# esw0116/DynaVSR

Hardware: AMD Instinct MI355X
Metric: inner-loop frames/sec/GPU (EDVR-M x4, 5x3x180x320): forward leg = BASELINE.json configs[1]; the inner MAML step and the per-frame pipeline are `inner_step` / `per_frame_pipeline` (higher is better)
Workload: dtype f32; 1 GPU; EDVR-M x4 forward (PCD deformable alignment + TSA fusion + reconstruction), clips of 1x5x3x180x320 -> 3x720x1280 (BASELINE.json configs[1]); one step = 2 clip(s) per GPU, one per HIP stream (adapt.super_resolve_video); clips_in_flight_per_gpu=2

## Files before the change

### dynavsr_amd/_lib.py

```python
import ctypes
import os
from ctypes import POINTER, Structure, c_char_p, c_float, c_int, c_longlong, c_size_t, c_void_p

import torch

_runtime = {"configured": False, "hw_queues": None, "effective": None}


def configure_runtime(hw_queues=6):
    if not _runtime["configured"]:
        user = os.environ.get("GPU_MAX_HW_QUEUES")
        late = torch.cuda.is_initialized()
        if user is None and not late:
            os.environ["GPU_MAX_HW_QUEUES"] = str(int(hw_queues))
        _runtime.update(configured=True, hw_queues=os.environ.get("GPU_MAX_HW_QUEUES"),
                        effective=(user is not None) or not late)
    return {"hw_queues": _runtime["hw_queues"], "effective": _runtime["effective"]}


def runtime_report(device=None):
    r = configure_runtime()
    overlaps = None
    if torch.cuda.is_available():
        with torch.cuda.device(device if device is not None else torch.cuda.current_device()):
            overlaps = int(lib().dvsr_side_stream_overlaps(stream()))
    return {"hw_queues": r["hw_queues"], "effective": r["effective"], "side_stream_overlaps": overlaps}


_HERE = os.path.dirname(os.path.abspath(__file__))
SO_PATH = os.path.join(_HERE, "libdynavsr_hip.so")
_lib = None

ACT_NONE, ACT_LRELU, ACT_RELU = 0, 1, 2


class Conv2dDesc(Structure):
    _fields_ = [("x0", c_void_p), ("x1", c_void_p), ("w", c_void_p), ("bias", c_void_p),
                ("res", c_void_p), ("y", c_void_p),
                ("N", c_int), ("c0", c_int), ("c1", c_int), ("H", c_int), ("W", c_int),
                ("Cout", c_int), ("ks", c_int), ("stride", c_int), ("pad", c_int), ("act", c_int),
                ("pixel_shuffle", c_int), ("x1_bdiv", c_int),
                ("x0_bstride", c_longlong), ("x1_bstride", c_longlong),
                ("pre", c_void_p), ("pre_bdiv", c_int)]


class EdvrConfig(Structure):
    _fields_ = [(k, c_int) for k in ("nf", "nframes", "groups", "front_RBs", "back_RBs", "scale",
                                     "center", "bf16_mfma")]


class FrameDesc(Structure):
    _fields_ = [("format", c_int), ("h", c_int), ("w", c_int), ("row_stride", c_longlong), ("plane_stride", c_longlong),
                ("pixel_stride", c_int)]


FRAME_F32_CHW, FRAME_U8_HWC_RGB, FRAME_U8_HWC_BGR, FRAME_U8_Y = 0, 1, 2, 3
FRAME_U16_Y_MSB, FRAME_U16_Y_10, FRAME_U16_Y_12 = 4, 5, 6
FRAME_PAD_REFLECT, FRAME_PAD_REPLICATE = 0, 1


class YuvDesc(Structure):
    _fields_ = [("format", c_int), ("h", c_int), ("w", c_int), ("matrix", c_int), ("range", c_int),
                ("plane", c_void_p * 3), ("row_stride", c_longlong * 3)]


YUV_NV12, YUV_I420 = 0, 1
YUV_BT601, YUV_BT709 = 0, 1
YUV_LIMITED, YUV_FULL = 0, 1


class Yuv16Desc(Structure):
    _fields_ = [("format", c_int), ("depth", c_int), ("h", c_int), ("w", c_int), ("matrix", c_int), ("range", c_int),
                ("plane", c_void_p * 3), ("row_stride", c_longlong * 3)]


YUV16_SEMI_MSB, YUV16_PLANAR_LSB = 0, 1


class ResizeAxis(Structure):
    _fields_ = [("first", c_void_p), ("weights", c_void_p), ("taps", c_int)]


FLIP_W, FLIP_H = 1, 2


class EstimatorConfig(Structure):
    _fields_ = [(k, c_int) for k in ("kind", "nf", "in_nc", "scale", "nframes")]


def _declare(lib):
    P, I, F, LL = c_void_p, c_int, c_float, c_longlong
    sig = {
        "dvsr_last_error": (c_char_p, []),
        "dvsr_version": (I, []),
        "dvsr_mdcn_forward": (I, [P] * 6 + [I] * 13 + [P]),
        "dvsr_mdcn_forward_fast_workspace_bytes": (c_size_t, [I, I, I]),
        "dvsr_mdcn_forward_fast": (I, [P] * 6 + [I] * 7 + [P, c_size_t, P]),
        "dvsr_mdcn_pack_forward": (I, [P] * 5 + [I] * 13 + [P]),
        "dvsr_conv2d_forward": (I, [POINTER(Conv2dDesc), P]),
        "dvsr_upsample_bilinear_forward": (I, [P, P, LL, I, I, I, F, P]),
        "dvsr_upsample_bilinear_backward": (I, [P, P, LL, I, I, I, F, I, P]),
        "dvsr_pool3s2_forward": (I, [P, P, P, LL, I, I, P]),
        "dvsr_pool3s2_backward": (I, [P, P, P, P, LL, I, I, P]),
        "dvsr_tsa_gate_forward": (I, [P] * 5 + [I, I, I, LL, P]),
        "dvsr_tsa_gate_backward": (I, [P] * 8 + [I, I, I, LL, P]),
        "dvsr_tsa_blend_forward": (I, [P] * 4 + [LL, P]),
        "dvsr_tsa_blend_backward": (I, [P] * 5 + [LL, P]),
        "dvsr_edvr_plan_create": (I, [POINTER(EdvrConfig), I, I, I, POINTER(c_void_p)]),
        "dvsr_edvr_plan_create_grouped": (I, [POINTER(EdvrConfig), I, I, I, I, POINTER(c_void_p)]),
        "dvsr_edvr_plan_create_ex": (I, [POINTER(EdvrConfig), I, I, I, I, I, POINTER(c_void_p)]),
        "dvsr_edvr_plan_destroy": (None, [P]),
        "dvsr_edvr_num_params": (I, [P]),
        "dvsr_edvr_num_launches": (I, [P]),
        "dvsr_edvr_workspace_bytes": (c_size_t, [P, I]),
        "dvsr_edvr_forward": (I, [P, POINTER(c_void_p), P, P, P, c_size_t, P]),
        "dvsr_edvr_forward_packed": (I, [P, POINTER(c_void_p), P, P, P, c_size_t, P]),
        "dvsr_edvr_backward": (I, [P, POINTER(c_void_p), P, P, POINTER(c_void_p), P, P, c_size_t, P]),
        "dvsr_edvr_num_backward_launches": (I, [P]),
        "dvsr_estimator_plan_create": (I, [POINTER(EstimatorConfig), I, I, I, POINTER(c_void_p)]),
        "dvsr_estimator_plan_create_grouped": (I, [POINTER(EstimatorConfig), I, I, I, I, POINTER(c_void_p)]),
        "dvsr_estimator_plan_create_ex": (I, [POINTER(EstimatorConfig), I, I, I, I, I, POINTER(c_void_p)]),
        "dvsr_estimator_plan_destroy": (None, [P]),
        "dvsr_estimator_num_params": (I, [P]),
        "dvsr_estimator_num_launches": (I, [P, I]),
        "dvsr_estimator_workspace_bytes": (c_size_t, [P, I]),
        "dvsr_estimator_forward": (I, [P, POINTER(c_void_p), P, P, P, c_size_t, P]),
        "dvsr_estimator_backward": (I, [P, POINTER(c_void_p), P, P, POINTER(c_void_p), P, c_size_t, P]),
        "dvsr_conv2d_backward_workspace_bytes": (c_size_t, [POINTER(Conv2dDesc)]),
        "dvsr_conv2d_backward": (I, [POINTER(Conv2dDesc), P, P, P, P, P, P, c_size_t, P]),
        "dvsr_mdcn_backward_workspace_bytes": (c_size_t, [I] * 10),
        "dvsr_mdcn_backward": (I, [P] * 10 + [I] * 12 + [P, c_size_t, P]),
        "dvsr_adam_step": (I, [POINTER(c_void_p)] * 4 + [POINTER(LL), I, F, F, F, F, F, I, P]),
        "dvsr_sgd_step": (I, [POINTER(c_void_p)] * 2 + [POINTER(LL), I, F, F, P]),
        "dvsr_replicate_tensors": (I, [POINTER(c_void_p)] * 2 + [POINTER(LL), I, I, P]),
        "dvsr_degrade_apply": (I, [P, P, P, I, I, I, I, I, I, I, I, I, P]),
        "dvsr_frame_metrics_workspace_bytes": (c_size_t, [I, I, I]),
        "dvsr_frame_metrics": (I, [P, P, I, I, I, F, F, P, P, P, c_size_t, P]),
        "dvsr_charbonnier_workspace_bytes": (c_size_t, []),
        "dvsr_charbonnier_forward": (I, [P, P, P, LL, F, P, c_size_t, P]),
        "dvsr_conv2d_packed_workspace_bytes": (c_size_t, [POINTER(Conv2dDesc)]),
        "dvsr_conv2d_forward_packed": (I, [POINTER(Conv2dDesc), P, c_size_t, P]),
        "dvsr_conv2d_dgrad_packed": (I, [POINTER(Conv2dDesc), P, P, P, c_size_t, P]),
        "dvsr_conv2d_packed_geometry": (I, [POINTER(Conv2dDesc), POINTER(ctypes.c_int * 4)]),
        "dvsr_conv2d_wgrad_geometry": (I, [POINTER(Conv2dDesc), I, I, POINTER(ctypes.c_int * 8)]),
        "dvsr_conv2d_wgrad_workspace_bytes": (c_size_t, [POINTER(Conv2dDesc), I]),
        "dvsr_conv2d_wgrad_bf16": (I, [POINTER(Conv2dDesc), P, P, P, P, c_size_t, P]),
        "dvsr_conv2d_wgrad_split3": (I, [POINTER(Conv2dDesc), P, P, P, P, c_size_t, P]),
        "dvsr_flow_warp_forward": (I, [P, P, P, I, I, I, I, LL, P]),
        "dvsr_flow_warp_backward": (I, [P, P, P, P, P, I, I, I, I, LL, P]),
        "dvsr_avgpool2_forward": (I, [P, P, LL, I, I, P]),
        "dvsr_avgpool2_backward": (I, [P, P, LL, I, I, I, P]),
        "dvsr_resize_bilinear_ac_forward": (I, [P, P, LL, I, I, I, I, F, LL, P]),
        "dvsr_resize_bilinear_ac_backward": (I, [P, P, LL, I, I, I, I, F, LL, P]),
        "dvsr_upsample_bicubic_ac_forward": (I, [P, P, LL, I, I, I, P]),
        "dvsr_upsample_bicubic_ac_backward": (I, [P, P, LL, I, I, I, P]),
        "dvsr_channel_affine": (I, [P, P, P, P, I, I, LL, LL, LL, I, P]),
        "dvsr_batchnorm_workspace_bytes": (c_size_t, [I]),
        "dvsr_batchnorm_forward": (I, [P] * 8 + [I, I, LL, I, F, F, I, P, c_size_t, P]),
        "dvsr_batchnorm_backward": (I, [P] * 9 + [I, I, LL, I, I, P, c_size_t, P]),
        "dvsr_temporal_gather3_forward": (I, [P, P, I, I, I, LL, I, P]),
        "dvsr_temporal_gather3_backward": (I, [P, P, I, I, I, LL, I, P]),
        "dvsr_dynamic_filter_forward": (I, [P, P, P, P, I, I, I, I, I, P]),
        "dvsr_dynamic_filter_backward": (I, [P, P, P, P, P, P, I, I, I, I, I, P]),
        "dvsr_conv3x3_small_cout": (I, [P, P, P, P, P, I, I, I, I, I, I, P]),
        "dvsr_conv1x1_dual": (I, [P, P, P, P, P, P, P, I, I, I, I, I, P]),
        "dvsr_patch_gather_forward": (I, [P, P, POINTER(c_int), POINTER(c_int), I, I, I, I, I, I, P]),
        "dvsr_patch_gather_backward": (I, [P, P, POINTER(c_int), POINTER(c_int), I, I, I, I, I, I, P]),
        "dvsr_l1_tail_forward": (I, [P, P, P, F, P, LL, P, c_size_t, P]),
        "dvsr_l1_tail_backward": (I, [P, P, P, F, P, LL, P]),
        "dvsr_charbonnier_backward": (I, [P, P, P, P, LL, F, P]),
        "dvsr_charbonnier_forward_grouped": (I, [P, P, P, LL, I, F, P, c_size_t, P]),
        "dvsr_charbonnier_backward_grouped": (I, [P, P, P, P, LL, I, F, P]),
        "dvsr_l1_tail_forward_grouped": (I, [P, P, P, F, P, LL, I, P, c_size_t, P]),
        "dvsr_l1_tail_backward_grouped": (I, [P, P, P, F, P, LL, I, P]),
        "dvsr_edvr_op_info": (I, [P, I, c_char_p, I, c_char_p, I, POINTER(ctypes.c_double),
                                  POINTER(ctypes.c_double)]),
        "dvsr_edvr_forward_timed": (I, [P, POINTER(c_void_p), P, P, P, c_size_t, P, POINTER(c_float)]),
        "dvsr_debug_mfma_peak": (LL, [P, I, I, I, I, P]),
        "dvsr_debug_mfma_shadow": (I, [P, P, I, I, I, I, I, P]),
        "dvsr_edvr_tensor_info": (I, [P, c_char_p, POINTER(LL), POINTER(LL)]),
        "dvsr_edvr_plan_work": (I, [P, POINTER(ctypes.c_double * 9)]),
        "dvsr_edvr_plan_work_nograd": (I, [P, POINTER(ctypes.c_double * 9)]),
        "dvsr_edvr_op_launch_count": (I, [P, I, I]),
        "dvsr_side_stream_overlaps": (I, [P]),
        "dvsr_edvr_op_output": (I, [P, I, I, POINTER(c_int), POINTER(LL), POINTER(LL)]),
        "dvsr_estimator_plan_work": (I, [P, POINTER(ctypes.c_double * 9)]),
        "dvsr_edvr_stream_create": (I, [POINTER(EdvrConfig), I, I, I, POINTER(c_void_p)]),
        "dvsr_edvr_stream_destroy": (None, [P]),
        "dvsr_edvr_stream_num_params": (I, [P]),
        "dvsr_edvr_stream_num_launches": (I, [P, I]),
        "dvsr_edvr_stream_cache_bytes": (c_size_t, [P]),
        "dvsr_edvr_stream_workspace_bytes": (c_size_t, [P]),
        "dvsr_edvr_stream_extract": (I, [P, POINTER(c_void_p), P, I, P, c_size_t, P, c_size_t, I, P]),
        "dvsr_edvr_stream_fuse": (I, [P, POINTER(c_void_p), POINTER(c_int), P, c_size_t, P, P, c_size_t, I, P]),
        "dvsr_frame_ingest": (I, [P, POINTER(FrameDesc), P, I, I, I, P]),
        "dvsr_frame_emit": (I, [P, I, I, P, POINTER(FrameDesc), F, F, P]),
        "dvsr_edvr_stream_extract_frame": (I, [P, POINTER(c_void_p), P, POINTER(FrameDesc), I, I, P, c_size_t, P, c_size_t, I,
                                               P]),
        "dvsr_frame_ingest_yuv": (I, [POINTER(YuvDesc), P, I, I, I, P]),
        "dvsr_frame_emit_yuv": (I, [P, I, I, POINTER(YuvDesc), F, F, P]),
        "dvsr_edvr_stream_extract_frame_yuv": (I, [P, POINTER(c_void_p), POINTER(YuvDesc), I, I, P, c_size_t, P, c_size_t, I, P]),
        "dvsr_frame_luma_sad": (I, [P, P, POINTER(FrameDesc), LL, I, P, P]),
        "dvsr_frame_ingest_yuv16": (I, [POINTER(Yuv16Desc), P, I, I, I, P]),
        "dvsr_frame_emit_yuv16": (I, [P, I, I, POINTER(Yuv16Desc), F, F, P]),
        "dvsr_edvr_stream_extract_frame_yuv16": (I, [P, POINTER(c_void_p), POINTER(Yuv16Desc), I, I, P, c_size_t, P, c_size_t, I,
                                                     P]),
        "dvsr_frame_resize_taps": (I, [I, I]),
        "dvsr_frame_resize_table": (I, [I, I, I, P, P]),
        "dvsr_frame_resize": (I, [P, I, I, I, I, P, I, I, I, I, POINTER(ResizeAxis), POINTER(ResizeAxis), P]),
        "dvsr_frame_flip": (I, [P, P, LL, I, I, I, P]),
        "dvsr_frame_flip_mean": (I, [P, P, P, P, P, LL, I, I, P]),
    }
    for name, (res, args) in sig.items():
        fn = getattr(lib, name)
        fn.restype = res
        fn.argtypes = args
    return sig


def lib():
    global _lib
    if _lib is None:
        if not os.path.exists(SO_PATH):
            raise RuntimeError(
                "libdynavsr_hip.so is missing (%s). Build it with `python -m dynavsr_amd.build` "
                "(hipcc --offload-arch=gfx950); there is no fallback path." % SO_PATH)
        _lib = ctypes.CDLL(os.environ.get("DVSR_HIP_LIB", SO_PATH))
        _lib._signatures = _declare(_lib)
    return _lib


def check(rc, what=""):
    if rc != 0:
        msg = lib().dvsr_last_error().decode("utf-8", "replace")
        raise RuntimeError("libdynavsr_hip %s failed (rc=%d): %s" % (what, rc, msg))


def ptr(t):
    if t is None:
        return None
    if not t.is_cuda:
        raise RuntimeError("libdynavsr_hip needs a tensor on the GPU, got device %s" % t.device)
    if t.dtype != torch.float32:
        raise RuntimeError("libdynavsr_hip computes in fp32, got %s" % t.dtype)
    if not t.is_contiguous():
        raise RuntimeError("libdynavsr_hip needs contiguous tensors")
    return t.data_ptr()


def stream():
    return torch.cuda.current_stream().cuda_stream
```

### dynavsr_amd/csrc/conv_small.hip

```cpp
#include "common.h"
#include "kernels.h"

namespace dvsr {

struct SmallK {
  const float* x; const float* w; const float* bias; const float* res; float* y;
  int N, C, H, W, Cout, act, tiles_x, tiles_y, ntiles;
  int wdiv; long long w_gs; int b_gs;
};

typedef float f32x2 __attribute__((ext_vector_type(2)));

template <int COUT>
__global__ __launch_bounds__(256) void conv3x3_small_cout_kernel(SmallK a) {
  constexpr int CC = 8, TH = 8, TW = 64, IH = TH + 2, IW = TW + 2, PLANE = IH * IW, E = (PLANE + 255) / 256;
  constexpr int WPC = ((9 * COUT + 3) / 4) * 4;
  __shared__ __attribute__((aligned(16))) float s_in[2][CC * PLANE];
  extern __shared__ __attribute__((aligned(16))) float s_w[];
  const int tpx = (a.ntiles + 7) >> 3;
  const int tile = (blockIdx.x & 7) * tpx + (blockIdx.x >> 3);
  if ((int)(blockIdx.x >> 3) >= tpx || tile >= a.ntiles) return;
  const int tx_ = tile % a.tiles_x;
  const int t2 = tile / a.tiles_x;
  const int ty_ = t2 % a.tiles_y;
  const int n = t2 / a.tiles_y;
  const int oy0 = ty_ * TH, ox0 = tx_ * TW;
  const int tid = threadIdx.x;
  const int py = tid >> 5, px2 = (tid & 31) * 2;
  const size_t HW = (size_t)a.H * a.W;
  const float* xn = a.x + (size_t)n * a.C * HW;
  const float* wn = wset_ptr(a.w, a.w_gs, n, a.wdiv);
  const float* bn = wset_ptr(a.bias, a.b_gs, n, a.wdiv);

  unsigned eoff[E];
  bool evalid[E];
#pragma unroll
  for (int e = 0; e < E; ++e) {
    const int idx = tid + 256 * e;
    const int iy = idx / IW, ix = idx - iy * IW;
    const int gy = oy0 - 1 + iy, gx = ox0 - 1 + ix;
    evalid[e] = idx < PLANE && (unsigned)gy < (unsigned)a.H && (unsigned)gx < (unsigned)a.W;
    eoff[e] = evalid[e] ? (unsigned)(gy * a.W + gx) * 4u : 0u;
  }
  f32x2 acc[COUT];
#pragma unroll
  for (int o = 0; o < COUT; ++o) acc[o] = f32x2{0.f, 0.f};
  float rin[CC][E];
  const int nch = ceil_div(a.C, CC);
  for (int i = tid; i < nch * CC * WPC; i += 256) {
    const int ci = i / WPC, r = i - ci * WPC;
    const int tap = r / COUT, o = r - tap * COUT;
    s_w[i] = (ci < a.C && tap < 9) ? wn[((size_t)o * a.C + ci) * 9 + tap] : 0.f;
  }
  auto prefetch = [&](int k) {
#pragma unroll
    for (int c = 0; c < CC; ++c) {
      const int ci = k * CC + c;
      const char* src = reinterpret_cast<const char*>(xn + (size_t)(ci < a.C ? ci : 0) * HW);
#pragma unroll
      for (int e = 0; e < E; ++e) rin[c][e] = *reinterpret_cast<const float*>(src + eoff[e]);
    }
  };
  prefetch(0);
  for (int k = 0; k < nch; ++k) {
    float* s = s_in[k & 1];
#pragma unroll
    for (int c = 0; c < CC; ++c)
#pragma unroll
      for (int e = 0; e < E; ++e) {
        const int idx = tid + 256 * e;
        if (e + 1 < E || idx < PLANE) s[c * PLANE + idx] = (evalid[e] && k * CC + c < a.C) ? rin[c][e] : 0.f;
      }
    __syncthreads();
    if (k + 1 < nch) prefetch(k + 1);
    const float* p0 = s + py * IW + px2;
#pragma unroll
    for (int c = 0; c < CC; ++c) {
      f32x4 wq[WPC / 4];
#pragma unroll
      for (int q = 0; q < WPC / 4; ++q)
        wq[q] = *reinterpret_cast<const f32x4*>(s_w + (size_t)(k * CC + c) * WPC + 4 * q);
#pragma unroll
      for (int ty = 0; ty < 3; ++ty) {
        const f32x2 lo = *reinterpret_cast<const f32x2*>(p0 + c * PLANE + ty * IW);
        const f32x2 hi = *reinterpret_cast<const f32x2*>(p0 + c * PLANE + ty * IW + 2);
        const float v[4] = {lo[0], lo[1], hi[0], hi[1]};
#pragma unroll
        for (int tx = 0; tx < 3; ++tx)
#pragma unroll
          for (int o = 0; o < COUT; ++o) {
            const int wi = (ty * 3 + tx) * COUT + o;
            const float wv = wq[wi >> 2][wi & 3];
            acc[o] = __builtin_elementwise_fma(f32x2{wv, wv}, f32x2{v[tx], v[tx + 1]}, acc[o]);
          }
      }
    }
  }
  const int oy = oy0 + py, ox = ox0 + px2;
  if (oy >= a.H || ox >= a.W) return;
  const bool two = ox + 1 < a.W;
  float bvs[COUT];
  f32x2 rvs[COUT];
#pragma unroll
  for (int o = 0; o < COUT; ++o) {
    bvs[o] = bn ? bn[o] : 0.f;
    const size_t idx = ((size_t)n * a.Cout + o) * HW + (size_t)oy * a.W + ox;
    rvs[o] = (a.res && two && (idx & 1) == 0) ? *reinterpret_cast<const f32x2*>(a.res + idx) : f32x2{0.f, 0.f};
  }
#pragma unroll
  for (int o = 0; o < COUT; ++o) {
    const float bv = bvs[o];
    f32x2 v = {apply_act(acc[o][0] + bv, a.act), apply_act(acc[o][1] + bv, a.act)};
    const size_t idx = ((size_t)n * a.Cout + o) * HW + (size_t)oy * a.W + ox;
    if (two && (idx & 1) == 0) {
      v += rvs[o];
      *reinterpret_cast<f32x2*>(a.y + idx) = v;
    } else {
      a.y[idx] = v[0] + (a.res ? a.res[idx] : 0.f);
      if (two) a.y[idx + 1] = v[1] + (a.res ? a.res[idx + 1] : 0.f);
    }
  }
}

struct SmallMfmaShape {
  static constexpr int TH = 6, TW = 56, RH = 8, RW = 64, X0 = 4, NPOS = RH * RW, APITCH = 68;
  static constexpr size_t LDS_BYTES = (size_t)(32 * APITCH + 27 * NPOS) * sizeof(float);
};

__device__ __forceinline__ __amdgpu_buffer_rsrc_t sm_rsrc(const float* base) {
  return __builtin_amdgcn_make_buffer_rsrc(const_cast<float*>(base), 0, 0x7fffffff, 0x00020000);
}
__device__ __forceinline__ f32x4 sm_load16(__amdgpu_buffer_rsrc_t rs, unsigned voff, unsigned soff) {
  return __builtin_bit_cast(f32x4, __builtin_amdgcn_raw_buffer_load_b128(rs, (int)voff, (int)soff, 0));
}

template <int COUT>
__global__ __launch_bounds__(256, 2) void conv3x3_small_cout_mfma_kernel(SmallK a) {
  using Sh = SmallMfmaShape;
  constexpr int TH = Sh::TH, TW = Sh::TW, RW = Sh::RW, NPOS = Sh::NPOS, AP = Sh::APITCH, NM = 9 * COUT;
  extern __shared__ __attribute__((aligned(16))) float s_mf[];
  float* const s_a = s_mf;
  float* const s_p = s_mf + 32 * AP;
  const int tpx = (a.ntiles + 7) >> 3;
  const int tile = (blockIdx.x & 7) * tpx + (blockIdx.x >> 3);
  if ((int)(blockIdx.x >> 3) >= tpx || tile >= a.ntiles) return;
  const int tx_ = tile % a.tiles_x;
  const int t2 = tile / a.tiles_x;
  const int ty_ = t2 % a.tiles_y;
  const int n = t2 / a.tiles_y;
  const int oy0 = ty_ * TH, ox0 = tx_ * TW;
  const int tid = threadIdx.x, lane = tid & 63;
  const int wave = __builtin_amdgcn_readfirstlane(tid >> 6);
  const int nn = lane & 31, kk = lane >> 5;
  const unsigned HW4 = (unsigned)a.H * a.W * 4u;
  const float* wn = wset_ptr(a.w, a.w_gs, n, a.wdiv);
  const float* bn = wset_ptr(a.bias, a.b_gs, n, a.wdiv);

  const int gy = oy0 - 1 + 2 * wave + (nn >> 4), gx = ox0 - Sh::X0 + 4 * (nn & 15);
  const bool inimg = (unsigned)gy < (unsigned)a.H && (unsigned)gx < (unsigned)a.W;
  const unsigned voff = inimg ? (unsigned)(8 * kk) * HW4 + (unsigned)(gy * a.W + gx) * 4u : 0x80000000u;
  const __amdgpu_buffer_rsrc_t xrs = sm_rsrc(a.x + (size_t)n * 64 * a.H * a.W);
  f32x4 B[2][16];
  auto issue = [&](int half) __attribute__((always_inline)) {
#pragma unroll
    for (int s = 0; s < 16; ++s) {
      const int c = 16 * (2 * half + (s >> 3)) + (s & 7);
      B[half][s] = sm_load16(xrs, voff, (unsigned)c * HW4);
    }
  };
  issue(0);
  for (int i = tid; i < 32 * 64; i += 256) {
    const int m = i >> 6, c = i & 63;
    const int tap = m / COUT, o = m - tap * COUT;
    s_a[m * AP + c] = m < NM ? wn[((size_t)o * 64 + c) * 9 + tap] : 0.f;
  }
  issue(1);
  __syncthreads();
  f32x4 A[8];
#pragma unroll
  for (int q = 0; q < 8; ++q) A[q] = *reinterpret_cast<const f32x4*>(s_a + nn * AP + 16 * (q >> 1) + 8 * kk + 4 * (q & 1));

  f32x16 acc[4];
#pragma unroll
  for (int j = 0; j < 4; ++j)
#pragma unroll
    for (int r = 0; r < 16; ++r) acc[j][r] = 0.f;
#pragma unroll
  for (int half = 0; half < 2; ++half)
#pragma unroll
    for (int s = 0; s < 16; ++s) {
      const int ch = 2 * half + (s >> 3), i = s & 7;
      const float av = A[2 * ch + (i >> 2)][i & 3];
#pragma unroll
      for (int j = 0; j < 4; ++j) acc[j] = __builtin_amdgcn_mfma_f32_32x32x2f32(av, B[half][s][j], acc[j], 0, 0, 0);
    }

#pragma unroll
  for (int r = 0; r < 16; ++r) {
    const int m = (r & 3) + 8 * (r >> 2) + 4 * kk;
    if (m < NM)
      *reinterpret_cast<f32x4*>(s_p + m * NPOS + 128 * wave + 4 * nn) = f32x4{acc[0][r], acc[1][r], acc[2][r], acc[3][r]};
  }
  __syncthreads();

  if (tid >= TH * (TW / 2)) return;
  const int y = tid / (TW / 2), xp = (tid - y * (TW / 2)) * 2;
  const int oy = oy0 + y, ox = ox0 + xp;
  if (oy >= a.H || ox >= a.W) return;
  float s0[COUT], s1[COUT];
#pragma unroll
  for (int o = 0; o < COUT; ++o) { s0[o] = 0.f; s1[o] = 0.f; }
#pragma unroll
  for (int dy = 0; dy < 3; ++dy) {
    const float* row = s_p + (y + dy) * RW + xp + Sh::X0 - 1;
#pragma unroll
    for (int dx = 0; dx < 3; ++dx)
#pragma unroll
      for (int o = 0; o < COUT; ++o) {
        const float* pm = row + ((dy * 3 + dx) * COUT + o) * NPOS + dx;
        s0[o] += pm[0];
        s1[o] += pm[1];
      }
  }
  const size_t HW = (size_t)a.H * a.W;
#pragma unroll
  for (int o = 0; o < COUT; ++o) {
    const float bv = bn ? bn[o] : 0.f;
    f32x2 v = {apply_act(s0[o] + bv, a.act), apply_act(s1[o] + bv, a.act)};
    const size_t idx = ((size_t)n * a.Cout + o) * HW + (size_t)oy * a.W + ox;
    if (a.res) v += *reinterpret_cast<const f32x2*>(a.res + idx);
    *reinterpret_cast<f32x2*>(a.y + idx) = v;
  }
}

template <int COUT>
static int launch_small_mfma(SmallK k, hipStream_t st) {
  using Sh = SmallMfmaShape;
  k.tiles_x = ceil_div(k.W, Sh::TW); k.tiles_y = ceil_div(k.H, Sh::TH); k.ntiles = k.tiles_x * k.tiles_y * k.N;
  auto kern = conv3x3_small_cout_mfma_kernel<COUT>;
  static PerDeviceOnce once;
  set_dyn_lds_once(once, (const void*)kern, Sh::LDS_BYTES);
  hipLaunchKernelGGL(kern, dim3(8 * ceil_div(k.ntiles, 8)), dim3(256), Sh::LDS_BYTES, st, k);
  return check_launch("conv3x3_small_cout_mfma_kernel");
}

int conv3x3_small_cout_run(const float* x, const float* w, const float* bias, const float* res, float* y, int N,
                           int C, int H, int W, int Cout, int act, hipStream_t st, int wdiv, long long w_gs, int b_gs) {
  DVSR_REQUIRE(x && w && y && Cout >= 1 && Cout <= 4, DVSR_ERR_INVALID, "conv3x3_small_cout: bad argument");
  SmallK k;
  k.x = x; k.w = w; k.bias = bias; k.res = res; k.y = y; k.N = N; k.C = C; k.H = H; k.W = W; k.Cout = Cout; k.act = act;
  k.wdiv = wdiv > 0 ? wdiv : 1; k.w_gs = w_gs; k.b_gs = b_gs;
  static const bool mfma_on = [] { const char* v = getenv("DVSR_CONV_LAST_MFMA"); return v && v[0] == '1'; }();
  if (mfma_on && C == 64 && Cout <= 3 && W % 4 == 0 && (unsigned long long)C * H * W * 4 < 0x7fffffffull &&
      ((((uintptr_t)x | (uintptr_t)y | (uintptr_t)res) & 15) == 0) && w_gs % 4 == 0) {
    if (Cout == 1) return launch_small_mfma<1>(k, st);
    if (Cout == 2) return launch_small_mfma<2>(k, st);
    return launch_small_mfma<3>(k, st);
  }
  k.tiles_x = ceil_div(W, 64); k.tiles_y = ceil_div(H, 8); k.ntiles = k.tiles_x * k.tiles_y * N;
  auto wbytes = [&](int cout) { return (size_t)ceil_div(C, 8) * 8 * (((9 * cout + 3) / 4) * 4) * sizeof(float); };
  switch (Cout) {
    case 1: hipLaunchKernelGGL(conv3x3_small_cout_kernel<1>, dim3(8 * ceil_div(k.ntiles, 8)), dim3(256), wbytes(1), st, k); break;
    case 2: hipLaunchKernelGGL(conv3x3_small_cout_kernel<2>, dim3(8 * ceil_div(k.ntiles, 8)), dim3(256), wbytes(2), st, k); break;
    case 3: hipLaunchKernelGGL(conv3x3_small_cout_kernel<3>, dim3(8 * ceil_div(k.ntiles, 8)), dim3(256), wbytes(3), st, k); break;
    default: hipLaunchKernelGGL(conv3x3_small_cout_kernel<4>, dim3(8 * ceil_div(k.ntiles, 8)), dim3(256), wbytes(4), st, k); break;
  }
  return check_launch("conv3x3_small_cout_kernel");
}

}

extern "C" int dvsr_conv3x3_small_cout(const float* x, const float* w, const float* bias, const float* res, float* y, int N,
                                       int C, int H, int W, int Cout, int act, dvsr_stream_t stream) {
  DVSR_REQUIRE(N > 0 && C > 0 && H > 0 && W > 0, DVSR_ERR_INVALID, "conv3x3_small_cout: empty tensor");
  return dvsr::conv3x3_small_cout_run(x, w, bias, res, y, N, C, H, W, Cout, act, (hipStream_t)stream, 1, 0, 0);
}
```

### dynavsr_amd/csrc/engine.hip

```cpp
#include <algorithm>
#include <cstdlib>
#include <string>
#include <vector>

#include "common.h"
#include "kernels.h"
#include "small_grid.h"

namespace dvsr {

enum { SP_ARENA = 0, SP_INPUT = 1, SP_OUTPUT = 2, SP_NONE = 3 };
struct T {
  int space = SP_NONE;
  size_t off = 0, numel = 0;
  bool valid() const { return space != SP_NONE; }
};

enum OpType { OP_CONV, OP_DCN, OP_UP, OP_POOL, OP_GATE, OP_BLEND, OP_ADD, OP_PAD, OP_MEANSUB, OP_ADDMEAN };

struct Op {
  OpType type;
  const char* name = "";
  T x0, x1, res, y, y2;
  int pw = -1, pb = -1;
  int N = 0, c0 = 0, c1 = 0, H = 0, W = 0, Cout = 0, ks = 3, stride = 1, act = 0, ps = 0;
  int x1_bdiv = 1, dg = 8;
  int pad = -1;
  int pmode = 0, T = 1;
  int wmap = 0;
  size_t w2_off = 0;
  int no_dgrad = 0;
  int pad_out = 0;
  struct T ypad;
  int fused_into = -1;
  int dual = -1;
  long long x0_bs = 0, x1_bs = 0;
  int S = 1;
  float mul = 1.f;
  size_t planes = 0;
  int gB = 0, gN = 0, gC = 0;
  size_t gHW = 0;
  struct PackSlot { ConvGeo geo = {8, 8, 2}; size_t off = 0, floats = 0; };
  PackSlot dgrad[2], dcn_pack;
  enum LaunchRole { WHOLE, MAIN_PART, REF_PART };
  struct Launch { PackSlot pack; int c_off = 0, c = 0; LaunchRole role = WHOLE; };
  struct LaunchList {
    int n = 0; Launch l[2];
    const Launch* begin() const { return l; }
    const Launch* end() const { return l + n; }
    const Launch& primary() const { return l[n - 1]; }
  } launches[2];
  struct T pre;
};
enum FwdMode { FWD_GRAD = 0, FWD_NOGRAD = 1 };

enum { R_ACT = 0, R_GRAD = 1, R_X = 2, R_GX = 3, R_GOUT = 4, R_TMP = 5, R_NONE = 6 };
struct Ref {
  int space = R_NONE;
  size_t off = 0;
};
enum BType { B_MEMSET, B_COPYADD, B_ACT, B_WGRAD, B_DGRAD, B_REDUCE, B_DCN, B_UP, B_POOL, B_GATE, B_BLEND,
             B_PADFOLD, B_ADDMEAN, B_WUNMAP };
struct BOp {
  BType type;
  int fwd = -1;
  Ref a, b, c, d, e, f;
  size_t n = 0;
  int accum = 0, which = 0, cnt = 1, B = 0;
  int mask_op = -1;
  size_t ws_off = 0, ws_bytes = 0;
  long long bs = 0;
  size_t per = 0;
};

static inline int conv_pad(const Op& o) { return o.pad < 0 ? o.ks / 2 : o.pad; }
static inline int conv_out(const Op& o, int in) { return (in + 2 * conv_pad(o) - o.ks) / o.stride + 1; }

}

struct dvsr_edvr_plan {
  dvsr_edvr_config cfg;
  int B, H, W;
  int n_params = 0;
  size_t arena_floats = 0;
  std::vector<dvsr::Op> ops;
  std::vector<std::pair<std::string, dvsr::T>> named;
  std::vector<std::pair<size_t, size_t>> allocs;
  std::vector<dvsr::BOp> bops;
  size_t dpack_floats = 0;
  bool use_v1 = false;
  size_t tmp_floats = 0;
  size_t scratch_bytes = 0;
  size_t wscratch_bytes = 0;
  mutable hipStream_t side = nullptr;
  mutable hipEvent_t ev_fork = nullptr, ev_join = nullptr;
  int side_streams = 1;
  int fork_every = 3;
  const char* bwd_unsupported = nullptr;
  int wgroups = 1;
  int wsets = 1;
  bool split_any_pad = false;
};

namespace dvsr {

static T arena_alloc(dvsr_edvr_plan& p, const char* name, size_t numel) {
  T t;
  t.space = SP_ARENA;
  t.off = p.arena_floats;
  t.numel = numel;
  p.allocs.emplace_back(t.off, numel);
  p.arena_floats += (numel + 63) & ~(size_t)63;
  if (name && *name) p.named.emplace_back(name, t);
  return t;
}

static WgradDesc wgrad_shape(const dvsr_edvr_plan& p, const Op& o, int which) {
  WgradDesc d;
  d.x_bs = which ? o.x1_bs : o.x0_bs; d.x_bdiv = which ? o.x1_bdiv : 1; d.gy_ps = o.ps;
  d.N = o.N; d.Cin = which ? o.c1 : o.c0; d.H = o.H; d.W = o.W; d.Cout = o.Cout;
  d.Ctot = o.c0 + o.c1; d.c_off = which ? o.c0 : 0;
  d.ks = o.ks; d.stride = o.stride; d.pad = conv_pad(o);
  d.groups = p.wgroups; d.dW_gs = (long long)o.Cout * (o.c0 + o.c1) * o.ks * o.ks; d.db_gs = o.Cout;
  d.mode = (p.cfg.bf16_mfma == 1 && !o.wmap) ? 1 : (wgrad_split3_default() ? 2 : 0);
  return d;
}

static Op::LaunchList plan_hoist(const Op& o, const dvsr_edvr_plan& p, ConvAllow fwd_ok, const Op::Launch& whole) {
  Op::LaunchList pair;
  const char* hv = getenv("DVSR_PCD_HOIST");
  if ((hv && hv[0] == '0') || p.use_v1 || p.wsets != 1 || whole.pack.geo.kernel != ConvKernel::WINO_F4 || o.x1_bdiv <= 1 || o.c1 <= 0 ||
      o.N % o.x1_bdiv != 0 || o.res.valid() || o.ps)
    return pair;
  const int Ho = conv_out(o, o.H), Wo = conv_out(o, o.W), bd = o.x1_bdiv;
  const ConvAllow shared = fwd_ok | ALLOW_WINO_F4 | ALLOW_SHARED_DEVICE;
  const ConvAllow only_f4 = without(fwd_ok, ALLOW_KSPLIT) | ALLOW_WINO_F4 | ALLOW_ONLY_F4;
  auto choose = [&](int n, int c, ConvAllow allow) { return conv2_choose(o.ks, o.stride, n, Ho, Wo, o.Cout, c, allow); };
  auto f4 = [](const ConvGeo& g) { return g.kernel == ConvKernel::WINO_F4; };
  const ConvGeo gm = choose(o.N, o.c0, shared), gr = choose(o.N / bd, o.c1, only_f4);
  const ConvGeo u1 = choose(bd, o.c0 + o.c1, shared), m1 = choose(bd, o.c0, shared), r1 = choose(1, o.c1, only_f4);
  if (f4(gm) && f4(gr) && f4(u1) && f4(m1) && f4(r1) &&
      conv2_f4_occupied_cycles(bd, Ho, Wo, o.Cout, o.c0, m1.th) + conv2_f4_occupied_cycles(1, Ho, Wo, o.Cout, o.c1, r1.th) <
          conv2_f4_occupied_cycles(bd, Ho, Wo, o.Cout, o.c0 + o.c1, u1.th)) {
    const size_t mf = conv2_pack_floats(o.ks, o.Cout, o.c0, gm), rf = conv2_pack_floats(o.ks, o.Cout, o.c1, gr);
    if (mf + rf <= whole.pack.floats)
      pair = {2, {{{gr, whole.pack.off + mf, rf}, o.c0, o.c1, Op::REF_PART}, {{gm, whole.pack.off, mf}, 0, o.c0, Op::MAIN_PART}}};
  }
  return pair;
}

static void plan_conv_launches(Op& o, dvsr_edvr_plan& p) {
  const int ks = o.ks, N = o.N, c0 = o.c0, c1 = o.c1, Cout = o.Cout, Ho = conv_out(o, o.H), Wo = conv_out(o, o.W);
  const char* s2 = getenv("DVSR_EST_SPLIT2");
  const int split2 = s2 ? atoi(s2) : 1;
  const bool bf = p.cfg.bf16_mfma && (ks == 3 || (ks == 2 && p.split_any_pad && p.cfg.bf16_mfma == 2 && split2 && c0 % 16 == 0)) &&
                  o.stride == 1 && (o.pad < 0 || p.split_any_pad) && (c1 == 0 || c0 % 16 == 0);
  static const int split_th8_from = getenv("DVSR_SPLIT_TH8_FROM") ? atoi(getenv("DVSR_SPLIT_TH8_FROM")) : 200;
  auto as_bf = [&](ConvGeo g, int ho, int wo, int cout, bool dgrad = false) {
    if (!bf || (ks == 2 && split2 == 2 && dgrad)) return g;
    if (ks == 2 && (long long)ceil_div(wo, 32) * ceil_div(ho, 4) * N * ceil_div(cout, 64) < 256) return g;
    g.cc = 16; g.th = 4; g.bf = p.cfg.bf16_mfma == 2 ? 2 : 1;
    if (g.bf == 2 && (long long)ceil_div(wo, 32) * ceil_div(ho, 8) * N * ceil_div(cout, 32 * g.mt) >= split_th8_from)
      g.th = 8;
    return g;
  };
  const bool plain = o.pad < 0 && !o.wmap && !p.cfg.bf16_mfma;
  const ConvAllow ks_ok = (plain && (c1 == 0 || c0 % 32 == 0) ? ALLOW_KSPLIT : ALLOW_NONE) |
                          (plain && c0 % 8 == 0 && c1 % 8 == 0 ? ALLOW_DMA_HALO | ALLOW_WINO : ALLOW_NONE);
  const ConvAllow fwd_ok = (o.ps == 0 || (o.ps == 2 && !o.res.valid())) ? ks_ok : without(ks_ok, ALLOW_WINO);
  auto whole = [&](const ConvGeo& g) {
    const size_t floats = conv2_pack_floats(ks, Cout, c0 + c1, g);
    return Op::Launch{{g, arena_alloc(p, "", floats * p.wsets).off, floats}, 0, c0 + c1, Op::WHOLE};
  };
  o.launches[FWD_GRAD] = {1, {whole(as_bf(conv2_choose(ks, o.stride, N, Ho, Wo, Cout, c0 + c1, fwd_ok), Ho, Wo, Cout))}};
  Op::LaunchList& nograd = o.launches[FWD_NOGRAD] = o.launches[FWD_GRAD];
  if ((fwd_ok & ALLOW_WINO) && !nograd.l[0].pack.geo.bf) {
    const ConvGeo g5 = conv2_choose(ks, o.stride, N, Ho, Wo, Cout, c0 + c1, fwd_ok | ALLOW_WINO_F4 | ALLOW_SHARED_DEVICE);
    if (g5.kernel == ConvKernel::WINO_F4) nograd.l[0] = whole(g5);
  }
  const Op::LaunchList pair = plan_hoist(o, p, fwd_ok, nograd.l[0]);
  if (pair.n) {
    o.pre = arena_alloc(p, "", (size_t)(N / o.x1_bdiv) * Cout * Ho * Wo);
    nograd = pair;
  }
  for (int which = 0; which < 2; ++which) {
    const int ci = which ? c1 : c0;
    if (!ci) continue;
    Op::PackSlot& dg = o.dgrad[which];
// ... 71 lines not shown

enum PlanPart { PART_WHOLE = 0, PART_EXTRACT = 1, PART_FUSE = 2 };

struct SlotLayout { size_t off[3], numel[3], raw, floats; };
static SlotLayout slot_layout(int C, int H, int W) {
  auto up = [](size_t n) { return (n + 63) & ~(size_t)63; };
  SlotLayout s;
  s.numel[0] = (size_t)C * H * W; s.numel[1] = (size_t)C * (H / 2) * (W / 2); s.numel[2] = (size_t)C * (H / 4) * (W / 4);
  s.off[0] = 0; s.off[1] = up(s.numel[0]); s.off[2] = s.off[1] + up(s.numel[1]);
  s.raw = s.off[2] + up(s.numel[2]);
  s.floats = s.raw + up((size_t)3 * H * W);
  return s;
}

static int build_plan(dvsr_edvr_plan& p, PlanPart part = PART_WHOLE) {
  const dvsr_edvr_config& c = p.cfg;
  const int B = p.B, Nf = c.nframes, C = c.nf, H = p.H, W = p.W, BN = B * Nf, dg = c.groups;
  const int H2 = H / 2, W2 = W / 2, H4 = H / 4, W4 = W / 4;
  const size_t HW = (size_t)H * W, HW2 = (size_t)H2 * W2, HW4 = (size_t)H4 * W4;
  Builder b(p);
  const int L = ACT_LRELU, R = ACT_RELU, NO = ACT_NONE;
  T none;
  const int EN = part == PART_EXTRACT ? 1 : BN;
  T xin; xin.space = SP_INPUT; xin.off = 0; xin.numel = (size_t)EN * 3 * HW;

  T f1, f2, f3;
  if (part == PART_FUSE) {
    f1 = b.alloc("L1_fea", (size_t)BN * C * HW);
    f2 = b.alloc("L2_fea", (size_t)BN * C * HW2);
    f3 = b.alloc("L3_fea", (size_t)BN * C * HW4);
    b.pcur += 2 * (1 + 2 * c.front_RBs + 4);
  } else {
    const SlotLayout sl = slot_layout(C, H, W);
    auto dst = [&](int l, bool final_of_level) {
      T t;
      if (part == PART_EXTRACT && final_of_level) { t.space = SP_OUTPUT; t.off = sl.off[l]; t.numel = sl.numel[l]; }
      return t;
    };
    f1 = b.conv("conv_first", b.take(), xin, 3, none, 0, EN, H, W, C, 3, 1, L, none, 0, 1, 0, 0, dst(0, c.front_RBs == 0));
    for (int i = 0; i < c.front_RBs; ++i) {
      auto p1 = b.take(); auto p2 = b.take();
      T t = b.conv("fe_rb_a", p1, f1, C, none, 0, EN, H, W, C, 3, 1, R);
      f1 = b.conv("fe_rb_b", p2, t, C, none, 0, EN, H, W, C, 3, 1, NO, f1, 0, 1, 0, 0, dst(0, i == c.front_RBs - 1));
    }
    p.named.emplace_back("L1_fea", f1);
    f2 = b.conv("fea_L2_conv1", b.take(), f1, C, none, 0, EN, H, W, C, 3, 2, L);
    f2 = b.conv("L2_fea", b.take(), f2, C, none, 0, EN, H2, W2, C, 3, 1, L, none, 0, 1, 0, 0, dst(1, true));
    f3 = b.conv("fea_L3_conv1", b.take(), f2, C, none, 0, EN, H2, W2, C, 3, 2, L);
    f3 = b.conv("L3_fea", b.take(), f3, C, none, 0, EN, H4, W4, C, 3, 1, L, none, 0, 1, 0, 0, dst(2, true));
  }
  if (part == PART_EXTRACT) {
    p.n_params = b.pcur;
    return DVSR_OK;
  }

  struct DP { int w, b; Builder::CP com; };
  auto take_dcn = [&]() { DP d; d.w = b.pcur; d.b = b.pcur + 1; b.pcur += 2; d.com = b.take(); return d; };
  auto L3o1 = b.take(); auto L3o2 = b.take(); DP L3d = take_dcn();
  auto L2o1 = b.take(); auto L2o2 = b.take(); auto L2o3 = b.take(); DP L2d = take_dcn(); auto L2f = b.take();
  auto L1o1 = b.take(); auto L1o2 = b.take(); auto L1o3 = b.take(); DP L1d = take_dcn(); auto L1f = b.take();
  auto cso1 = b.take(); auto cso2 = b.take(); DP csd = take_dcn();
  const int ctr = c.center;
  T ref1 = Builder::view(f1, (size_t)ctr * C * HW, 0), ref2 = Builder::view(f2, (size_t)ctr * C * HW2, 0),
    ref3 = Builder::view(f3, (size_t)ctr * C * HW4, 0);
  const long long rs1 = (long long)Nf * C * HW, rs2 = (long long)Nf * C * HW2, rs3 = (long long)Nf * C * HW4;
  T o3 = b.conv("L3_offset_conv1", L3o1, f3, C, ref3, C, BN, H4, W4, C, 3, 1, L, none, 0, Nf, 0, rs3);
  o3 = b.conv("L3_offset", L3o2, o3, C, none, 0, BN, H4, W4, C, 3, 1, L);
  T om3 = b.conv("L3_om", L3d.com, o3, C, none, 0, BN, H4, W4, dg * 27, 3, 1, NO);
  T fe3 = b.dcn("L3_aligned", L3d.w, L3d.b, f3, om3, BN, C, H4, W4, dg, L);
  T o2 = b.conv("L2_offset_conv1", L2o1, f2, C, ref2, C, BN, H2, W2, C, 3, 1, L, none, 0, Nf, 0, rs2);
  T u3 = b.up("L3_offset_up", o3, (size_t)BN * C, H4, W4, 2, 2.f);
  o2 = b.conv("L2_offset_conv2", L2o2, o2, C, u3, C, BN, H2, W2, C, 3, 1, L);
  o2 = b.conv("L2_offset", L2o3, o2, C, none, 0, BN, H2, W2, C, 3, 1, L);
  T om2 = b.conv("L2_om", L2d.com, o2, C, none, 0, BN, H2, W2, dg * 27, 3, 1, NO);
  T d2 = b.dcn("L2_dcn", L2d.w, L2d.b, f2, om2, BN, C, H2, W2, dg, NO);
  T uf3 = b.up("L3_aligned_up", fe3, (size_t)BN * C, H4, W4, 2, 1.f);
  T fe2 = b.conv("L2_aligned", L2f, d2, C, uf3, C, BN, H2, W2, C, 3, 1, L);
  T o1 = b.conv("L1_offset_conv1", L1o1, f1, C, ref1, C, BN, H, W, C, 3, 1, L, none, 0, Nf, 0, rs1);
  T u2 = b.up("L2_offset_up", o2, (size_t)BN * C, H2, W2, 2, 2.f);
  o1 = b.conv("L1_offset_conv2", L1o2, o1, C, u2, C, BN, H, W, C, 3, 1, L);
  o1 = b.conv("L1_offset", L1o3, o1, C, none, 0, BN, H, W, C, 3, 1, L);
  T om1 = b.conv("L1_om", L1d.com, o1, C, none, 0, BN, H, W, dg * 27, 3, 1, NO);
  T d1 = b.dcn("L1_dcn", L1d.w, L1d.b, f1, om1, BN, C, H, W, dg, NO);
  T uf2 = b.up("L2_aligned_up", fe2, (size_t)BN * C, H2, W2, 2, 1.f);
  T fe1 = b.conv("L1_aligned", L1f, d1, C, uf2, C, BN, H, W, C, 3, 1, NO);
  T oc = b.conv("cas_offset_conv1", cso1, fe1, C, ref1, C, BN, H, W, C, 3, 1, L, none, 0, Nf, 0, rs1);
  oc = b.conv("cas_offset", cso2, oc, C, none, 0, BN, H, W, C, 3, 1, L);
  T omc = b.conv("cas_om", csd.com, oc, C, none, 0, BN, H, W, dg * 27, 3, 1, NO);
  T aligned = b.dcn("aligned", csd.w, csd.b, fe1, omc, BN, C, H, W, dg, L);

  auto tA1 = b.take(); auto tA2 = b.take(); auto ffu = b.take(); auto s1 = b.take(); auto s2 = b.take();
  auto s3 = b.take(); auto s4 = b.take(); auto s5 = b.take(); auto sL1 = b.take(); auto sL2 = b.take();
  auto sL3 = b.take(); auto sa1 = b.take(); auto sa2 = b.take();
  T emb_ref = b.conv("tsa_emb_ref", tA2, Builder::view(aligned, (size_t)ctr * C * HW, 0), C, none, 0, B, H,
                     W, C, 3, 1, NO, none, 0, 1, (long long)Nf * C * HW);
  T emb = b.conv("tsa_emb", tA1, aligned, C, none, 0, BN, H, W, C, 3, 1, NO);
  T cor = b.alloc("tsa_cor", (size_t)BN * HW);
  T gated = b.alloc("tsa_gated", (size_t)BN * C * HW);
  {
    Op o; o.type = OP_GATE; o.name = "tsa_gate"; o.x0 = emb; o.x1 = emb_ref; o.res = aligned;
    o.y = cor; o.y2 = gated; o.gB = B; o.gN = Nf; o.gC = C; o.gHW = HW;
    p.ops.push_back(o);
  }
  T fea = b.conv("tsa_fea", ffu, gated, Nf * C, none, 0, B, H, W, C, 1, 1, L);
  T att = b.conv("tsa_att1", s1, gated, Nf * C, none, 0, B, H, W, C, 1, 1, L);
  {
    static const bool dual_on = [] { const char* v = getenv("DVSR_TSA_DUAL"); return !(v && v[0] == '0'); }();
    const int ia = (int)p.ops.size() - 2, ib = ia + 1;
    if (dual_on && C == 64 && !p.cfg.bf16_mfma) { p.ops[ia].dual = ib; p.ops[ib].fused_into = ia; }
  }
  T pmx, pav;
  b.pool("tsa_pool1", att, (size_t)B * C, H, W, pmx, pav);
  att = b.conv("tsa_att2", s2, pmx, C, pav, C, B, H2, W2, C, 1, 1, L);
  T attL = b.conv("tsa_attL1", sL1, att, C, none, 0, B, H2, W2, C, 1, 1, L);
  T qmx, qav;
  b.pool("tsa_pool2", attL, (size_t)B * C, H2, W2, qmx, qav);
  attL = b.conv("tsa_attL2", sL2, qmx, C, qav, C, B, H4, W4, C, 3, 1, L);
  attL = b.conv("tsa_attL3", sL3, attL, C, none, 0, B, H4, W4, C, 3, 1, L);
  T attLu = b.up("tsa_attL_up", attL, (size_t)B * C, H4, W4, 2, 1.f);
  T a3 = b.conv("tsa_att3", s3, att, C, none, 0, B, H2, W2, C, 3, 1, L);
  T att3 = b.alloc("tsa_att3_sum", (size_t)B * C * HW2);
  {
    Op o; o.type = OP_ADD; o.name = "tsa_att3_add"; o.x0 = a3; o.x1 = attLu; o.y = att3;
    p.ops.push_back(o);
  }
  T a4 = b.conv("tsa_att4", s4, att3, C, none, 0, B, H2, W2, C, 1, 1, L);
  T a4u = b.up("tsa_att4_up", a4, (size_t)B * C, H2, W2, 2, 1.f);
  T a5 = b.conv("tsa_att", s5, a4u, C, none, 0, B, H, W, C, 3, 1, NO);
  T ad = b.conv("tsa_add1", sa1, a5, C, none, 0, B, H, W, C, 1, 1, L);
  ad = b.conv("tsa_add2", sa2, ad, C, none, 0, B, H, W, C, 1, 1, NO);
  T out = b.alloc("tsa_out", (size_t)B * C * HW);
  {
    Op o; o.type = OP_BLEND; o.name = "tsa_blend"; o.x0 = fea; o.x1 = a5; o.res = ad; o.y = out;
    p.ops.push_back(o);
  }

  for (int i = 0; i < c.back_RBs; ++i) {
    auto p1 = b.take(); auto p2 = b.take();
    T t = b.conv("rc_rb_a", p1, out, C, none, 0, B, H, W, C, 3, 1, R);
    out = b.conv("rc_rb_b", p2, t, C, none, 0, B, H, W, C, 3, 1, NO, out);
  }
  p.named.emplace_back("recon", out);
  int h = H, w = W;
  if (c.scale == 4) {
    out = b.conv("upconv1", b.take(), out, C, none, 0, B, h, w, C * 4, 3, 1, L, none, 2);
    h *= 2; w *= 2;
    out = b.conv("upconv2", b.take(), out, C, none, 0, B, h, w, 256, 3, 1, L, none, 2);
  } else {
    out = b.conv("upconv2", b.take(), out, C, none, 0, B, h, w, 256, 3, 1, L, none, 2);
  }
  h *= 2; w *= 2;
  out = b.conv("HRconv", b.take(), out, 64, none, 0, B, h, w, 64, 3, 1, L);
  T base = b.alloc("base", (size_t)B * 3 * h * w);
  for (int bi = 0; bi < B; ++bi) {
    Op o; o.type = OP_UP; o.name = "base_up";
    o.x0 = Builder::view(xin, part == PART_FUSE ? 0 : ((size_t)bi * Nf + ctr) * 3 * HW, 3 * HW);
    o.planes = 3; o.H = H; o.W = W; o.S = c.scale; o.mul = 1.f;
    o.y = Builder::view(base, (size_t)bi * 3 * h * w, (size_t)3 * h * w);
    p.ops.push_back(o);
  }
  T yout; yout.space = SP_OUTPUT; yout.off = 0; yout.numel = (size_t)B * 3 * h * w;
  b.conv("conv_last", b.take(), out, 64, none, 0, B, h, w, 3, 3, 1, NO, base, 0, 1, 0, 0, yout);
  p.n_params = b.pcur;
  return DVSR_OK;
}


struct BackBuilder {
  dvsr_edvr_plan& p;
  std::vector<char> written;
  struct Pending { Ref src; size_t n; int fwd; };
  std::vector<Pending> pending;
  bool gx_zeroed = false;
  explicit BackBuilder(dvsr_edvr_plan& plan) : p(plan), written(plan.allocs.size(), 0), pending(plan.allocs.size()) {}

  int alloc_index(size_t off) const {
    int lo = 0, hi = (int)p.allocs.size() - 1, ans = -1;
    while (lo <= hi) {
      const int mid = (lo + hi) / 2;
      if (p.allocs[mid].first <= off) { ans = mid; lo = mid + 1; } else hi = mid - 1;
    }
    return ans;
  }
  static Ref act(const T& t) {
    Ref r;
    r.space = t.space == SP_ARENA ? R_ACT : (t.space == SP_INPUT ? R_X : R_NONE);
    r.off = t.off;
    return r;
  }
  static Ref grad(const T& t) {
    Ref r;
    r.space = t.space == SP_ARENA ? R_GRAD : (t.space == SP_INPUT ? R_GX : (t.space == SP_OUTPUT ? R_GOUT : R_NONE));
    r.off = t.off;
    return r;
  }
  void materialize(int ai) {
    if (ai < 0 || written[ai] != 2) return;
    BOp o;
    o.type = B_COPYADD; o.fwd = pending[ai].fwd; o.a.space = R_GRAD; o.a.off = p.allocs[ai].first; o.b = pending[ai].src;
    o.n = pending[ai].n; o.accum = 0;
    p.bops.push_back(o);
    written[ai] = 1;
  }
  void materialize(const T& t) { if (t.space == SP_ARENA) materialize(alloc_index(t.off)); }
  bool take_pending_as_residual(const T& t, Ref* src) {
    if (t.space != SP_ARENA) return false;
    const int ai = alloc_index(t.off);
    if (written[ai] != 2 || t.off != p.allocs[ai].first || t.numel != p.allocs[ai].second || pending[ai].n != t.numel)
      return false;
    *src = pending[ai].src;
    written[ai] = 1;
    return true;
  }
  int contribute(const T& t, bool full, int fwd) {
    if (t.space == SP_INPUT) return 1;
    const int ai = alloc_index(t.off);
    const bool whole = full && t.off == p.allocs[ai].first && t.numel == p.allocs[ai].second;
    materialize(ai);
    if (written[ai]) return 1;
    written[ai] = 1;
    if (whole) return 0;
    BOp m;
    m.type = B_MEMSET; m.fwd = fwd; m.a.space = R_GRAD; m.a.off = p.allocs[ai].first; m.n = p.allocs[ai].second;
    p.bops.push_back(m);
    return 1;
  }
  void copyadd(const T& dst, const Ref& src, size_t n, int fwd) {
    if (dst.space == SP_ARENA) {
      const int ai = alloc_index(dst.off);
      static const bool defer = [] { const char* v = getenv("DVSR_FUSE_RES_BWD"); return !(v && v[0] == '0'); }();
      if (defer && !written[ai] && dst.off == p.allocs[ai].first && dst.numel == p.allocs[ai].second && n == dst.numel) {
        written[ai] = 2;
        pending[ai] = Pending{src, n, fwd};
        return;
      }
    }
    BOp o;
    o.type = B_COPYADD; o.fwd = fwd; o.a = grad(dst); o.b = src; o.n = n;
    o.accum = contribute(dst, true, fwd);
    p.bops.push_back(o);
  }
};

static int sole_producer_with_act(const dvsr_edvr_plan& p, const T& t, int consumer) {
  if (t.space != SP_ARENA) return -1;
  int prod = -1;
  for (int j = 0; j < consumer; ++j) {
    const Op& q = p.ops[j];
    if (q.type == OP_CONV && q.act != ACT_NONE && q.y.space == SP_ARENA && q.y.off == t.off && q.y.numel == t.numel &&
        !q.ps)
      prod = j;
  }
  if (prod < 0) return -1;
  const Op& q = p.ops[prod];
  int readers = 0;
  for (size_t j = 0; j < p.ops.size(); ++j) {
    const Op& r = p.ops[j];
    for (const T* in : {&r.x0, &r.x1, &r.res})
      if (in->space == SP_ARENA && in->off < q.y.off + q.y.numel && in->off + in->numel > q.y.off) ++readers;
  }
  return readers == 1 ? prod : -1;
}

static void build_backward(dvsr_edvr_plan& p) {
  BackBuilder bb(p);
  size_t tmp = 0, scratch = 0, wscratch = 0;
  std::vector<char> act_fused(p.ops.size(), 0);
  const bool fuse_act = !p.use_v1 && [] { const char* v = getenv("DVSR_FUSE_ACT_BWD"); return !(v && v[0] == '0'); }();
  for (int i = (int)p.ops.size() - 1; i >= 0; --i) {
    const Op& o = p.ops[i];
    const Ref gy = BackBuilder::grad(o.y);
    bb.materialize(o.y);
    bb.materialize(o.y2);
    if (o.type == OP_GATE) bb.materialize(o.res);
    switch (o.type) {
      case OP_CONV: {
        if (o.res.valid() && o.act != ACT_NONE) p.bwd_unsupported = "a convolution with both a residual input and an activation";
        if (o.res.valid()) bb.copyadd(o.res, gy, o.y.numel, i);
        if (o.act != ACT_NONE && !act_fused[i]) {
          BOp a; a.type = B_ACT; a.fwd = i; a.a = gy; a.b = BackBuilder::act(o.y); a.n = o.y.numel;
          p.bops.push_back(a);
        }
        for (int which = 0; which < 2; ++which) {
          if (which == 1 && !o.c1) break;
          BOp w; w.type = B_WGRAD; w.fwd = i; w.which = which; w.a = BackBuilder::act(which ? o.x1 : o.x0); w.b = gy;
          p.bops.push_back(w);
          BOp& wr = p.bops.back();
          wr.ws_bytes = (conv2d_wgrad_workspace_bytes(wgrad_shape(p, o, which)) + 255) & ~(size_t)255;
          wr.ws_off = wscratch;
          wscratch += wr.ws_bytes;
          if (o.wmap) {
            BOp u; u.type = B_WUNMAP; u.fwd = i;
            p.bops.push_back(u);
          }
        }
        for (int which = 0; which < 2; ++which) {
          if ((which == 1 && !o.c1) || o.no_dgrad) break;
          const T& xin = which ? o.x1 : o.x0;
          const int ci = which ? o.c1 : o.c0;
          const bool strided = which ? (o.x1_bdiv > 1 || o.x1_bs != 0) : (o.x0_bs != 0);
          BOp d; d.type = B_DGRAD; d.fwd = i; d.which = which; d.b = gy;
          if (!strided) {
            T full = xin; full.numel = (size_t)o.N * ci * o.H * o.W;
            if (!p.use_v1 && bb.take_pending_as_residual(full, &d.e)) d.accum = 0;
            else d.accum = bb.contribute(full, true, i);
            d.a = BackBuilder::grad(xin);
            if (!d.accum && !o.c1 && fuse_act && d.e.space == R_NONE) {
              const int prod = sole_producer_with_act(p, full, i);
              if (prod >= 0) { d.mask_op = prod; act_fused[prod] = 1; }
            }
            p.bops.push_back(d);
          } else {
            d.accum = 0; d.a.space = R_TMP; d.a.off = 0;
            p.bops.push_back(d);
            const int bdiv = which ? o.x1_bdiv : 1;
// ... 128 lines not shown
  g.ks = o->ks; g.stride = 1; g.pad = o->ks - 1 - conv_pad(*o); g.act = ACT_NONE; g.x1_bdiv = 1;
  g.res = bs.at(b.e);
  ConvExtra ex;
  ex.wt = 1; ex.w_ctot = o->c0 + o->c1; ex.w_coff = b.which ? o->c0 : 0; ex.accum = b.accum; ex.in_ps = o->ps ? 1 : 0;
  if (b.mask_op >= 0 && !p.use_v1) { ex.gmask = bs.arena + p.ops[b.mask_op].y.off; ex.gmask_act = p.ops[b.mask_op].act; }
  if (o->stride == 2) { ex.in_dil = 2; ex.Hs = Ho; ex.Ws = Wo; g.H = o->H; g.W = o->W; }
  else { g.H = Ho; g.W = Wo; }
  set_wsets(p, o->N, o->dgrad[b.which].floats, 0, &ex);
  *gd = g; *exd = ex;
}

static int run_backward_op(const dvsr_edvr_plan& p, const BOp& b, const float* const* P, float* const* GP,
                           const BBases& bs, void* scratch, size_t scratch_bytes, hipStream_t st) {
  const Op* o = b.fwd >= 0 ? &p.ops[b.fwd] : nullptr;
  switch (b.type) {
    case B_MEMSET: {
      hipError_t e = hipMemsetAsync(bs.at(b.a), 0, b.n * sizeof(float), st);
      DVSR_REQUIRE(e == hipSuccess, DVSR_ERR_HIP, "backward memset: %s", hipGetErrorString(e));
      return DVSR_OK;
    }
    case B_COPYADD: {
      float* dst = bs.at(b.a);
      if (!dst) return DVSR_OK;
      if (b.accum) return add_inplace(dst, bs.at(b.b), b.n, st);
      hipError_t e = hipMemcpyAsync(dst, bs.at(b.b), b.n * sizeof(float), hipMemcpyDeviceToDevice, st);
      DVSR_REQUIRE(e == hipSuccess, DVSR_ERR_HIP, "backward copy: %s", hipGetErrorString(e));
      return DVSR_OK;
    }
    case B_ACT:
      return act_bwd_inplace(bs.at(b.a), bs.at(b.b), b.n, o->act, st);
    case B_WUNMAP:
      return w4_to_s2d(bs.garena + o->w2_off, GP[o->pw], p.wgroups * o->Cout, o->c0 / 4, 1, st);
    case B_PADFOLD: {
      float* gx = bs.at(b.a);
      if (!gx) return DVSR_OK;
      const bool mpad = b.mask_op >= 0 && p.ops[b.mask_op].pad_out;
      return pad_bwd(bs.at(b.b), gx, o->pmode, o->N, o->c0, o->H, o->W, o->T, b.accum, st,
                     b.mask_op >= 0 ? bs.arena + (mpad ? o->y.off : p.ops[b.mask_op].y.off) : nullptr,
                     b.mask_op >= 0 ? p.ops[b.mask_op].act : 0, mpad ? 1 : 0);
    }
    case B_ADDMEAN:
      return addmean_bwd(bs.at(b.b), bs.at(b.a), o->N / o->T, o->c0, o->T, (size_t)o->H * o->W, st);
    case B_DGRAD: {
      if (!bs.at(b.a)) return DVSR_OK;
      dvsr_conv2d_desc g;
      ConvExtra ex;
      dgrad_desc(p, b, P, bs, &g, &ex);
      if (p.use_v1) return conv2d_run(g, ex, st);
      return conv2d_packed_run(g, bs.dpack + o->dgrad[b.which].off, ex, o->dgrad[b.which].geo, st);
    }
    case B_REDUCE: {
      float* dst = bs.at(b.a);
      if (!dst) return DVSR_OK;
      return reduce_frames(dst, b.bs, bs.at(b.b), b.B, b.cnt, b.per, b.accum, st);
    }
    case B_DCN: {
      const size_t P_ = (size_t)o->H * o->W;
      const long long bstride = (long long)o->dg * 27 * P_;
      const float* om = bs.arena + o->x1.off;
      float* gom = bs.at(b.c);
      return mdcn_backward_run(bs.arena + o->x0.off, om, bstride, om + (size_t)o->dg * 18 * P_, bstride, 1, P[o->pw],
                               bs.at(b.b), bs.at(b.a), gom, bstride, gom + (size_t)o->dg * 18 * P_, bstride,
                               GP[o->pw], GP[o->pb], o->N, o->c0, o->H, o->W, o->Cout, 1, 1, 1, o->dg, scratch,
                               scratch_bytes, st, p.wgroups, (long long)o->Cout * o->c0 * 9, o->Cout,
                               p.wsets > 1 ? (long long)o->Cout * o->c0 * 9 : 0);
    }
    case B_UP: {
      float* gx = bs.at(b.a);
      if (!gx) return DVSR_OK;
      return upsample_bilinear_bwd(bs.at(b.b), gx, o->planes, o->H, o->W, o->S, o->mul, b.accum, st);
    }
    case B_POOL:
      return pool3s2_bwd(bs.arena + o->x0.off, bs.at(b.b), bs.at(b.c), bs.at(b.a), o->planes, o->H, o->W, b.accum, st);
    case B_GATE:
      return tsa_gate_bwd(bs.arena + o->x0.off, bs.arena + o->x1.off, bs.arena + o->res.off, bs.arena + o->y.off,
                          bs.at(b.b), bs.at(b.a), bs.at(b.c), bs.at(b.d), o->gB, o->gN, o->gC, o->gHW, st,
                          bs.garena + o->y.off);
    case B_BLEND:
      return tsa_blend_bwd(bs.arena + o->x0.off, bs.arena + o->x1.off, bs.at(b.b), bs.at(b.a), bs.at(b.c),
                           o->y.numel, b.accum, st);
    case B_WGRAD: break;
  }
  return DVSR_ERR_INVALID;
}

struct Bases {
  float* arena; const float* x; float* out;
  FwdMode mode;
  float* at(const T& t) const {
    if (t.space == SP_ARENA) return arena + t.off;
    if (t.space == SP_INPUT) return const_cast<float*>(x) + t.off;
    if (t.space == SP_OUTPUT) return out + t.off;
    return nullptr;
  }
};

static int pack_all(const dvsr_edvr_plan& p, const float* const* P, float* arena_base, float* fwd_base,
                    float* bwd_base, hipStream_t st, FwdMode mode = FWD_GRAD) {
  PackTable t;
  t.n = 0;
  auto flush = [&]() { int rc = pack_weights_run(t, st); t.n = 0; return rc; };
  const int S = p.wsets;
  for (const Op& o : p.ops) {
    if (o.type == OP_DCN && fwd_base && o.dcn_pack.floats) {
      for (int ws = 0; ws < S; ++ws) {
        t.e[t.n++] = conv2_pack_entry(P[o.pw] + (size_t)ws * o.Cout * o.c0 * 9, fwd_base + o.dcn_pack.off + (size_t)ws * o.dcn_pack.floats,
                                      3, o.Cout, o.c0, 8, 0, mdcn_pack_layout(o.W));
        if (t.n == 48) { int rc = flush(); if (rc) return rc; }
      }
    }
    if (o.type != OP_CONV) continue;
    const int ctot = o.c0 + o.c1, KK = o.ks * o.ks;
    const size_t wnum = (size_t)o.Cout * ctot * KK;
    const float* wsrc = P[o.pw];
    if (o.wmap) {
      wsrc = arena_base + o.w2_off;
      if (fwd_base) {
        int rc = w4_to_s2d(P[o.pw], arena_base + o.w2_off, S * o.Cout, ctot / 4, 0, st);
        if (rc) return rc;
      }
    }
    for (int ws = 0; ws < S; ++ws) {
      if (fwd_base) {
        for (const Op::Launch& l : o.launches[mode]) {
          const bool sliced = l.c != ctot;
          t.e[t.n++] = conv2_pack_entry(wsrc + ws * wnum, fwd_base + l.pack.off + (size_t)ws * l.pack.floats, o.ks, o.Cout, l.c, l.pack.geo,
                                        0, sliced ? ctot : 0, sliced ? l.c_off : 0);
          if (t.n == 48) { int rc = flush(); if (rc) return rc; }
        }
      }
      if (bwd_base) {
        for (int which = 0; which < 2; ++which) {
          const int ci = which ? o.c1 : o.c0;
          if (!ci) continue;
          const Op::PackSlot& dg = o.dgrad[which];
          t.e[t.n++] = conv2_pack_entry(wsrc + ws * wnum, bwd_base + dg.off + (size_t)ws * dg.floats, o.ks, ci, o.Cout, dg.geo, 1, ctot,
                                        which ? o.c0 : 0);
          if (t.n == 48) { int rc = flush(); if (rc) return rc; }
        }
      }
    }
  }
  return flush();
}

static dvsr_conv2d_desc launch_desc(dvsr_conv2d_desc d, const Op& o, Op::LaunchRole role, float* pre) {
  if (role == Op::WHOLE) return d;
  if (role == Op::REF_PART) { d.x0 = d.x1; d.c0 = o.c1; d.x0_bstride = o.x1_bs; d.N = o.N / o.x1_bdiv; d.act = ACT_NONE; d.y = pre; }
  else { d.bias = nullptr; d.pre = pre; d.pre_bdiv = o.x1_bdiv; }
  d.x1 = nullptr; d.c1 = 0; d.x1_bdiv = 1; d.x1_bstride = 0;
  return d;
}

static int run_forward_op(const dvsr_edvr_plan& p, const Op& o, const float* const* P, const Bases& bs, hipStream_t st) {
  switch (o.type) {
    case OP_CONV: {
      dvsr_conv2d_desc d = {};
      d.x0 = bs.at(o.x0); d.x1 = bs.at(o.x1); d.w = P[o.pw]; d.bias = P[o.pb]; d.res = bs.at(o.res);
      d.y = bs.at(o.y);
      d.N = o.N; d.c0 = o.c0; d.c1 = o.c1; d.H = o.H; d.W = o.W; d.Cout = o.Cout; d.ks = o.ks;
      d.stride = o.stride; d.pad = conv_pad(o); d.act = o.act; d.pixel_shuffle = o.ps;
      if (o.pad_out) { d.y = bs.at(o.ypad); d.pixel_shuffle = o.pad_out; }
      if (!p.use_v1 && (o.dual >= 0 || o.fused_into >= 0)) {
        const Op& oa = o.dual >= 0 ? o : p.ops[o.fused_into];
        const Op& ob = p.ops[oa.dual];
        const long long HW = (long long)oa.H * oa.W;
        auto plain1x1 = [](const Op& q) {
          return q.type == OP_CONV && q.ks == 1 && q.stride == 1 && q.c1 == 0 && q.Cout == 64 && !q.res.valid() && !q.ps && !q.wmap && !q.pad_out;
        };
        const bool pair_ok = plain1x1(oa) && plain1x1(ob) && oa.act == ob.act && oa.c0 == ob.c0 && oa.N == ob.N && oa.H == ob.H &&
                             oa.W == ob.W && oa.x0.space == ob.x0.space && oa.x0.off == ob.x0.off;
        if (pair_ok && conv1x1_dual_ok(bs.at(oa.x0), P[oa.pw], P[ob.pw], bs.at(oa.y), bs.at(ob.y), oa.c0, HW)) {
          if (o.fused_into >= 0) return DVSR_OK;
          return conv1x1_dual_run(bs.at(oa.x0), P[oa.pw], P[oa.pb], P[ob.pw], P[ob.pb], bs.at(oa.y), bs.at(ob.y), oa.N, oa.c0,
                                  (int)HW, oa.act, st, p.wsets > 1 ? oa.N / p.wsets : 1,
                                  p.wsets > 1 ? (long long)oa.Cout * oa.c0 : 0, p.wsets > 1 ? oa.Cout : 0);
        }
      }
      if (o.wmap) d.w = bs.arena + o.w2_off;
      d.x1_bdiv = o.x1_bdiv; d.x0_bstride = o.x0_bs; d.x1_bstride = o.x1_bs;
      if (p.use_v1) return conv2d_run(d, ConvExtra(), st);
      if (o.Cout <= 4 && o.ks == 3 && o.stride == 1 && !o.c1 && !o.ps && !o.x0_bs && o.pad < 0)
        return conv3x3_small_cout_run(d.x0, d.w, d.bias, d.res, d.y, o.N, o.c0, o.H, o.W, o.Cout, o.act, st,
                                      p.wsets > 1 ? o.N / p.wsets : 1, p.wsets > 1 ? (long long)o.Cout * o.c0 * 9 : 0,
                                      p.wsets > 1 ? o.Cout : 0);
      for (const Op::Launch& l : o.launches[bs.mode]) {
        ConvExtra ex;
        set_wsets(p, o.N, l.pack.floats, o.Cout, &ex);
        int rc = conv2d_packed_run(launch_desc(d, o, l.role, bs.at(o.pre)), bs.arena + l.pack.off, ex, l.pack.geo, st);
        if (rc != DVSR_OK) return rc;
      }
      return DVSR_OK;
    }
    case OP_DCN: {
      const float* om = bs.at(o.x1);
      const long long bstride = (long long)o.dg * 27 * o.H * o.W;
      if (!p.use_v1 && o.dcn_pack.floats)
        return mdcn_forward_packed_run(bs.at(o.x0), om, bstride, om + (size_t)o.dg * 18 * o.H * o.W, bstride, 1,
                                       bs.arena + o.dcn_pack.off, P[o.pb], bs.at(o.y), o.N, o.c0, o.H, o.W, o.Cout,
                                       o.dg, o.act, st, p.wsets > 1 ? o.N / p.wsets : 1,
                                       p.wsets > 1 ? (long long)o.dcn_pack.floats : 0, p.wsets > 1 ? o.Cout : 0, mdcn_pack_layout(o.W));
      return mdcn_forward_run(bs.at(o.x0), om, bstride, om + (size_t)o.dg * 18 * o.H * o.W, bstride, 1,
                              P[o.pw], P[o.pb], bs.at(o.y), o.N, o.c0, o.H, o.W, o.Cout, 3, 3, 1, 1,
                              1, 1, o.dg, o.act, st);
    }
    case OP_UP:
      return upsample_bilinear_fwd(bs.at(o.x0), bs.at(o.y), o.planes, o.H, o.W, o.S, o.mul, st);
    case OP_POOL:
      return pool3s2_fwd(bs.at(o.x0), bs.at(o.y), bs.at(o.y2), o.planes, o.H, o.W, st);
    case OP_GATE:
      return tsa_gate_fwd(bs.at(o.x0), bs.at(o.x1), bs.at(o.res), bs.at(o.y), bs.at(o.y2), o.gB, o.gN,
                          o.gC, o.gHW, st);
    case OP_BLEND:
      return tsa_blend_fwd(bs.at(o.x0), bs.at(o.x1), bs.at(o.res), bs.at(o.y), o.y.numel, st);
    case OP_PAD:
      if (o.fused_into >= 0) return DVSR_OK;
      return pad_fwd(bs.at(o.x0), bs.at(o.y), o.pmode, o.N, o.c0, o.H, o.W, o.T, st);
    case OP_MEANSUB:
      return meansub_fwd(bs.at(o.x0), bs.at(o.y), bs.at(o.y2), bs.at(o.res), o.N / o.T, o.c0, o.T, o.H, o.W, st);
    case OP_ADDMEAN:
      return addmean_fwd(bs.at(o.x0), bs.at(o.x1), bs.at(o.y), o.N / o.T, o.c0, o.T, (size_t)o.H * o.W, st);
    case OP_ADD:
      return add_out(bs.at(o.y), bs.at(o.x0), bs.at(o.x1), o.y.numel, st);
  }
  return DVSR_ERR_INVALID;
}

}

using namespace dvsr;

extern "C" int dvsr_edvr_plan_create(const dvsr_edvr_config* cfg, int B, int H, int W,
                                     dvsr_edvr_plan** out) {
  return dvsr_edvr_plan_create_grouped(cfg, B, H, W, 1, out);
}

extern "C" int dvsr_edvr_plan_create_grouped(const dvsr_edvr_config* cfg, int B, int H, int W, int grad_groups,
                                             dvsr_edvr_plan** out) {
  return dvsr_edvr_plan_create_ex(cfg, B, H, W, grad_groups, 1, out);
}

extern "C" int dvsr_edvr_plan_create_ex(const dvsr_edvr_config* cfg, int B, int H, int W, int grad_groups,
                                        int weight_sets, dvsr_edvr_plan** out) {
  DVSR_REQUIRE(cfg && out, DVSR_ERR_INVALID, "edvr_plan_create: null argument");
  DVSR_REQUIRE(weight_sets == 1 || weight_sets == grad_groups, DVSR_ERR_INVALID,
               "edvr_plan_create: weight_sets=%d must be 1 or grad_groups=%d", weight_sets, grad_groups);
  DVSR_REQUIRE(B > 0 && H > 0 && W > 0 && H % 4 == 0 && W % 4 == 0, DVSR_ERR_INVALID,
               "edvr_plan_create: B=%d H=%d W=%d (H, W must be positive multiples of 4)", B, H, W);
  DVSR_REQUIRE(grad_groups >= 1 && B % grad_groups == 0, DVSR_ERR_INVALID,
               "edvr_plan_create: grad_groups=%d must divide the batch B=%d", grad_groups, B);
  DVSR_REQUIRE(cfg->nf > 0 && cfg->nf % cfg->groups == 0 && cfg->nframes > 0 && cfg->front_RBs >= 0 &&
                   cfg->back_RBs >= 0, DVSR_ERR_INVALID, "edvr_plan_create: bad network config");
  DVSR_REQUIRE(cfg->scale == 4 || cfg->scale == 2, DVSR_ERR_UNSUPPORTED,
               "edvr_plan_create: scale=%d (2 or 4)", cfg->scale);
  DVSR_REQUIRE(cfg->center >= 0 && cfg->center < cfg->nframes, DVSR_ERR_INVALID,
               "edvr_plan_create: center=%d out of range", cfg->center);
  const int cpg = cfg->nf / cfg->groups;
  DVSR_REQUIRE(cpg == 4 || cpg == 8 || cpg == 16, DVSR_ERR_UNSUPPORTED,
               "edvr_plan_create: nf/groups=%d (supported: 4, 8, 16)", cpg);
  dvsr_edvr_plan* p = new dvsr_edvr_plan();
  p->cfg = *cfg; p->B = B; p->H = H; p->W = W; p->wgroups = grad_groups; p->wsets = weight_sets;
  { const char* v = getenv("DVSR_CONV_V1"); p->use_v1 = v && v[0] == '1'; }
  if (weight_sets > 1 && (p->use_v1 || cpg % 8 != 0)) {
    delete p;
    DVSR_REQUIRE(false, DVSR_ERR_UNSUPPORTED, "edvr_plan_create: per-sample weight sets need the packed kernels (no "
                 "DVSR_CONV_V1) and nf/groups a multiple of 8");
  }
  { const char* v = getenv("DVSR_BWD_STREAMS"); p->side_streams = (v && v[0] == '0') ? 0 : 1; }
  int rc = build_plan(*p);
  if (rc != DVSR_OK) { delete p; return rc; }
  build_backward(*p);
  *out = p;
  return DVSR_OK;
}

extern "C" void dvsr_edvr_plan_destroy(dvsr_edvr_plan* p) {
  if (!p) return;
  if (p->side) (void)hipStreamSynchronize(p->side);
  if (p->ev_fork) {
    (void)hipEventDestroy(p->ev_fork);
    (void)hipEventDestroy(p->ev_join);
  }
  delete p;
}

extern "C" int dvsr_edvr_num_params(const dvsr_edvr_plan* p) { return p ? p->n_params : -1; }

extern "C" int dvsr_edvr_num_launches(const dvsr_edvr_plan* p) { return p ? (int)p->ops.size() : -1; }

extern "C" size_t dvsr_edvr_workspace_bytes(const dvsr_edvr_plan* p, int need_grad) {
  if (!p) return 0;
  size_t b = p->arena_floats * sizeof(float);
  if (need_grad)
    b += (p->arena_floats + p->tmp_floats + p->dpack_floats) * sizeof(float) + p->scratch_bytes + p->wscratch_bytes;
  return b;
}

extern "C" int dvsr_edvr_backward(const dvsr_edvr_plan* p, const float* const* params, const float* x,
                                  const float* grad_out, float* const* grad_params, float* grad_x, void* ws,
                                  size_t ws_bytes, dvsr_stream_t stream) {
  DVSR_REQUIRE(p && params && x && grad_out && grad_params && ws, DVSR_ERR_INVALID, "edvr_backward: null argument");
  DVSR_REQUIRE(!p->bwd_unsupported, DVSR_ERR_UNSUPPORTED, "edvr_backward: the tape holds %s", p->bwd_unsupported);
  DVSR_REQUIRE(ws_bytes >= dvsr_edvr_workspace_bytes(p, 1), DVSR_ERR_WORKSPACE,
               "edvr_backward: workspace %zu < %zu bytes (allocate with need_grad=1 BEFORE the forward)", ws_bytes,
               dvsr_edvr_workspace_bytes(p, 1));
  hipStream_t st = (hipStream_t)stream;
  BBases bs;
  bs.arena = (float*)ws; bs.garena = bs.arena + p->arena_floats; bs.x = x; bs.gx = grad_x; bs.gout = grad_out;
  bs.tmp = bs.garena + p->arena_floats;
  bs.dpack = bs.tmp + p->tmp_floats;
  void* scratch = bs.dpack + p->dpack_floats;
  if (!p->use_v1) {
    int rc = pack_all(*p, params, bs.arena, nullptr, bs.dpack, st);
    if (rc != DVSR_OK) return rc;
  }
  if (grad_x) {
    const size_t n = (size_t)p->B * p->cfg.nframes * 3 * p->H * p->W;
    DVSR_REQUIRE(hipMemsetAsync(grad_x, 0, n * sizeof(float), st) == hipSuccess, DVSR_ERR_HIP,
                 "edvr_backward: memset of grad_x failed");
  }
  bool use_side = p->side_streams != 0;
  if (use_side && !p->ev_fork) {
    if (hipEventCreateWithFlags(&p->ev_fork, hipEventDisableTiming) != hipSuccess ||
        hipEventCreateWithFlags(&p->ev_join, hipEventDisableTiming) != hipSuccess) {
      (void)hipGetLastError();
      p->ev_fork = nullptr;
      use_side = false;
    }
  }
  if (use_side) {
    p->side = side_stream_for(st);
    if (!p->side) use_side = false;
  }
  void* wscratch = (char*)scratch + p->scratch_bytes;
  DVSR_REQUIRE(hipMemsetAsync(wscratch, 0, p->wscratch_bytes, st) == hipSuccess, DVSR_ERR_HIP,
               "edvr_backward: memset of the wgrad scratch failed");
  bool forked = false;
  int last_fork_fwd = -1;
  std::vector<WgradReduceEntry> reduces;
  std::vector<const BOp*> unmaps;
  reduces.reserve(p->bops.size());
  static const int fork_env = [] { const char* v = getenv("DVSR_BWD_FORK_EVERY"); return v ? atoi(v) : 0; }();
  const int fork_every = fork_env > 0 ? fork_env : p->fork_every;
  std::vector<WgradLaunch> waiting;
  int waiting_layers = 0;
  auto flush_waiting = [&]() -> int {
    if (waiting.empty()) return DVSR_OK;
    hipStream_t ws = st;
    if (use_side) {
      DVSR_REQUIRE(hipEventRecord(p->ev_fork, st) == hipSuccess && hipStreamWaitEvent(p->side, p->ev_fork, 0) == hipSuccess,
                   DVSR_ERR_HIP, "edvr_backward: fork to the wgrad stream failed");
      ws = p->side;
      forked = true;
    }
    for (const WgradLaunch& l : waiting) {
      int rc = conv2d_wgrad_launch(l, ws);
      if (rc != DVSR_OK) return rc;
    }
    waiting.clear();
    waiting_layers = 0;
    return DVSR_OK;
  };
  for (const BOp& b : p->bops) {
    int rc = DVSR_OK;
    if (b.type == B_WGRAD) {
      reduces.emplace_back();
      WgradLaunch l;
      rc = prep_wgrad(*p, b, grad_params, bs, (char*)wscratch + b.ws_off, b.ws_bytes, st, &reduces.back(), &l);
      if (rc != DVSR_OK) return rc;
      if (b.fwd != last_fork_fwd) {
        if (waiting_layers >= fork_every) rc = flush_waiting();
        last_fork_fwd = b.fwd;
        ++waiting_layers;
      }
      waiting.push_back(l);
      if (rc == DVSR_OK && (!use_side || !l.geo.row_split)) rc = flush_waiting();
    } else if (b.type == B_WUNMAP) {
      unmaps.push_back(&b);
    } else {
      rc = run_backward_op(*p, b, params, grad_params, bs, scratch, p->scratch_bytes, st);
    }
    if (rc != DVSR_OK) return rc;
  }
  {
    int rc = flush_waiting();
    if (rc != DVSR_OK) return rc;
    hipStream_t ws = use_side && forked ? p->side : st;
    rc = wgrad_reduce_batch(reduces.data(), (int)reduces.size(), ws);
    if (rc != DVSR_OK) return rc;
    for (const BOp* b : unmaps) {
      rc = run_backward_op(*p, *b, params, grad_params, bs, nullptr, 0, ws);
      if (rc != DVSR_OK) return rc;
    }
  }
  if (forked)
    DVSR_REQUIRE(hipEventRecord(p->ev_join, p->side) == hipSuccess &&
                     hipStreamWaitEvent(st, p->ev_join, 0) == hipSuccess,
                 DVSR_ERR_HIP, "edvr_backward: join of the wgrad stream failed");
  return DVSR_OK;
}

extern "C" int dvsr_edvr_num_backward_launches(const dvsr_edvr_plan* p) { return p ? (int)p->bops.size() : -1; }

static FwdMode forward_mode(const dvsr_edvr_plan* p, size_t ws_bytes) {
  return ws_bytes < dvsr_edvr_workspace_bytes(p, 1) ? FWD_NOGRAD : FWD_GRAD;
}

static int run_forward_tape(const dvsr_edvr_plan& p, const float* const* params, const Bases& bs, bool packs_valid, hipStream_t st) {
  if (!p.use_v1 && !packs_valid) {
    int rc = pack_all(p, params, bs.arena, bs.arena, nullptr, st, bs.mode);
    if (rc != DVSR_OK) return rc;
  }
  for (const Op& o : p.ops) {
    int rc = run_forward_op(p, o, params, bs, st);
    if (rc != DVSR_OK) return rc;
  }
  return DVSR_OK;
}

static int edvr_forward_impl(const dvsr_edvr_plan* p, const float* const* params, const float* x, float* out, void* ws,
                             size_t ws_bytes, dvsr_stream_t stream, bool packs_valid);

extern "C" int dvsr_edvr_forward(const dvsr_edvr_plan* p, const float* const* params, const float* x,
                                 float* out, void* ws, size_t ws_bytes, dvsr_stream_t stream) {
  return edvr_forward_impl(p, params, x, out, ws, ws_bytes, stream, false);
}

extern "C" int dvsr_edvr_forward_packed(const dvsr_edvr_plan* p, const float* const* params, const float* x,
                                        float* out, void* ws, size_t ws_bytes, dvsr_stream_t stream) {
  return edvr_forward_impl(p, params, x, out, ws, ws_bytes, stream, true);
}

static int edvr_forward_impl(const dvsr_edvr_plan* p, const float* const* params, const float* x, float* out, void* ws,
                             size_t ws_bytes, dvsr_stream_t stream, bool packs_valid) {
  DVSR_REQUIRE(p && params && x && out && ws, DVSR_ERR_INVALID, "edvr_forward: null argument");
  DVSR_REQUIRE(ws_bytes >= p->arena_floats * sizeof(float), DVSR_ERR_WORKSPACE,
               "edvr_forward: workspace %zu < %zu bytes", ws_bytes, p->arena_floats * sizeof(float));
  return run_forward_tape(*p, params, Bases{(float*)ws, x, out, forward_mode(p, ws_bytes)}, packs_valid, (hipStream_t)stream);
}

static void op_work(const Op& o, const char** kind, double* flops, double* bytes) {
  *flops = 0; *bytes = 0; *kind = "other";
  switch (o.type) {
    case OP_CONV: {
      const int Ho = conv_out(o, o.H), Wo = conv_out(o, o.W);
      const double ctot = o.c0 + o.c1, px = (double)o.N * Ho * Wo;
      *flops = 2.0 * px * o.Cout * ctot * o.ks * o.ks;
      *bytes = 4.0 * ((double)o.N * o.c0 * o.H * o.W + (double)(o.N / o.x1_bdiv) * o.c1 * o.H * o.W +
                      px * o.Cout * (o.res.valid() ? 2 : 1) + (double)o.Cout * ctot * o.ks * o.ks);
      *kind = o.ks == 1 ? "conv1x1" : (o.ks == 2 ? "conv2x2" : (o.stride == 2 ? "conv3x3s2" : "conv3x3s1"));
      break;
    }
    case OP_DCN: {
      const double px = (double)o.N * o.H * o.W;
      *flops = 2.0 * px * o.Cout * o.c0 * 9 + px * o.c0 * 9 * 8.0;
      *bytes = 4.0 * (px * o.c0 + px * o.dg * 27 + px * o.Cout + (double)o.Cout * o.c0 * 9);
      *kind = "mdcn";
      break;
    }
    case OP_UP: *bytes = 4.0 * o.planes * o.H * o.W * (1.0 + o.S * o.S); *kind = "upsample"; break;
    case OP_POOL: *bytes = 4.0 * o.planes * o.H * o.W * 1.5; *kind = "pool"; break;
    case OP_GATE: *bytes = 4.0 * ((double)o.gB * o.gN * o.gC * o.gHW * 3 + (double)o.gB * o.gC * o.gHW +
                                 (double)o.gB * o.gN * o.gHW); *kind = "tsa_gate"; break;
    case OP_BLEND: *bytes = 4.0 * o.y.numel * 4; *kind = "tsa_blend"; break;
    case OP_ADD: *bytes = 4.0 * o.y.numel * 3; *kind = "add"; break;
    case OP_PAD: *bytes = 4.0 * ((double)o.N * o.c0 * o.H * o.W + (double)o.y.numel); *kind = "pad"; break;
    case OP_MEANSUB: *bytes = 4.0 * o.y.numel * 3; *kind = "meansub"; break;
    case OP_ADDMEAN: *bytes = 4.0 * o.y.numel * 2; *kind = "addmean"; break;
  }
}

extern "C" int dvsr_edvr_op_info(const dvsr_edvr_plan* p, int index, char* kind, int kind_cap,
                                 char* name, int name_cap, double* flops, double* bytes) {
  DVSR_REQUIRE(p && kind && name && flops && bytes && index >= 0 && index < (int)p->ops.size(),
               DVSR_ERR_INVALID, "edvr_op_info: bad argument");
  const char* k;
  op_work(p->ops[index], &k, flops, bytes);
  snprintf(kind, kind_cap, "%s", k);
  if (p->ops[index].type == OP_CONV)
  {
    const ConvGeo& g = p->ops[index].launches[FWD_NOGRAD].primary().pack.geo;
    snprintf(name, name_cap, "%s[%d/%d/%d%s]", p->ops[index].name, g.cc, g.th, g.mt, kernel_tag(g.kernel));
  }
  else
    snprintf(name, name_cap, "%s", p->ops[index].name);
  return DVSR_OK;
}

extern "C" int dvsr_edvr_op_launch_count(const dvsr_edvr_plan* p, int index, int nograd) {
  if (!p || index < 0 || index >= (int)p->ops.size()) return -1;
  const Op& o = p->ops[index];
  return o.type == OP_CONV ? o.launches[nograd ? FWD_NOGRAD : FWD_GRAD].n : 1;
}

static int plan_work(const dvsr_edvr_plan* p, double* out9, FwdMode mode) {
  DVSR_REQUIRE(p && out9, DVSR_ERR_INVALID, "edvr_plan_work: null argument");
  double fa = 0, fe = 0, ba = 0, be = 0, fby = 0, f32p[2] = {0, 0}, bfp[2] = {0, 0};
  auto conv_part = [](const Op& o, int ci) {
    return 2.0 * (double)o.N * conv_out(o, o.H) * conv_out(o, o.W) * o.Cout * ci * o.ks * o.ks;
  };
  auto issue = [&](const ConvGeo& g, double f, double* ex, int pass) {
    const double shaped = f * multiplies_per_output_ratio(g.kernel);
    *ex += shaped;
    if (on_bf16_split(g.kernel) || g.bf == 2) bfp[pass] += 6.0 * shaped;
    else if (g.bf == 1) bfp[pass] += shaped;
    else f32p[pass] += shaped;
  };
  for (const Op& o : p->ops) {
    {
      const char* k; double fl, by;
      op_work(o, &k, &fl, &by);
      fby += by;
    }
    if (o.type == OP_CONV) {
      const double f = conv_part(o, o.c0 + o.c1);
      fa += f;
      for (const Op::Launch& l : o.launches[mode])
        issue(l.pack.geo, conv_part(o, l.c) / (l.role == Op::REF_PART ? o.x1_bdiv : 1), &fe, 0);
    } else if (o.type == OP_DCN) {
      const double f = 2.0 * (double)o.N * o.H * o.W * o.Cout * o.c0 * 9;
      fa += f; fe += f; f32p[0] += f;
    }
  }
  for (const BOp& b : p->bops) {
    if (b.fwd < 0) continue;
    const Op& o = p->ops[b.fwd];
    if (b.type == B_WGRAD) {
      const double f = conv_part(o, b.which ? o.c1 : o.c0);
      ba += f; be += f;
      const WgradKernel k = conv2d_wgrad_choose(wgrad_shape(*p, o, b.which)).kernel;
      if (on_bf16_split(k)) bfp[1] += 6.0 * f; else if (on_bf16_pipe(k)) bfp[1] += f; else f32p[1] += f;
    } else if (b.type == B_DGRAD) {
      const double f = conv_part(o, b.which ? o.c1 : o.c0);
      ba += f; issue(o.dgrad[b.which].geo, f, &be, 1);
    } else if (b.type == B_DCN) {
      const double f = 2.0 * 2.0 * (double)o.N * o.H * o.W * o.Cout * o.c0 * 9;
      ba += f; be += f; f32p[1] += f;
    }
  }
  out9[0] = fa; out9[1] = fe; out9[2] = ba; out9[3] = be;
  out9[4] = fby;
  out9[5] = f32p[0]; out9[6] = bfp[0]; out9[7] = f32p[1]; out9[8] = bfp[1];
  return DVSR_OK;
}
extern "C" int dvsr_edvr_plan_work(const dvsr_edvr_plan* p, double* out9) { return plan_work(p, out9, FWD_GRAD); }
extern "C" int dvsr_edvr_plan_work_nograd(const dvsr_edvr_plan* p, double* out9) { return plan_work(p, out9, FWD_NOGRAD); }

extern "C" int dvsr_edvr_forward_timed(const dvsr_edvr_plan* p, const float* const* params,
                                       const float* x, float* out, void* ws, size_t ws_bytes,
                                       dvsr_stream_t stream, float* op_ms) {
  DVSR_REQUIRE(p && params && x && out && ws && op_ms, DVSR_ERR_INVALID, "edvr_forward_timed: null argument");
  DVSR_REQUIRE(ws_bytes >= p->arena_floats * sizeof(float), DVSR_ERR_WORKSPACE,
               "edvr_forward_timed: workspace too small");
  hipStream_t st = (hipStream_t)stream;
  const size_t n = p->ops.size();
  std::vector<hipEvent_t> ev(n + 1);
  for (auto& e : ev) DVSR_REQUIRE(hipEventCreate(&e) == hipSuccess, DVSR_ERR_HIP, "hipEventCreate failed");
  const Bases bs{(float*)ws, x, out, forward_mode(p, ws_bytes)};
  int rc = p->use_v1 ? DVSR_OK : pack_all(*p, params, bs.arena, bs.arena, nullptr, st, bs.mode);
  hipEventRecord(ev[0], st);
  for (size_t i = 0; i < n && rc == DVSR_OK; ++i) {
    rc = run_forward_op(*p, p->ops[i], params, bs, st);
    hipEventRecord(ev[i + 1], st);
  }
  if (rc == DVSR_OK && hipStreamSynchronize(st) != hipSuccess) {
    set_error("edvr_forward_timed: stream synchronize failed");
    rc = DVSR_ERR_HIP;
  }
  if (rc == DVSR_OK)
    for (size_t i = 0; i < n; ++i) hipEventElapsedTime(&op_ms[i], ev[i], ev[i + 1]);
  for (auto& e : ev) hipEventDestroy(e);
  return rc;
}

extern "C" int dvsr_edvr_op_output(const dvsr_edvr_plan* p, int index, int which, int* in_arena, long long* offset_floats,
                                   long long* numel) {
  DVSR_REQUIRE(p && in_arena && offset_floats && numel && index >= 0 && index < (int)p->ops.size() && (which == 0 || which == 1),
               DVSR_ERR_INVALID, "edvr_op_output: bad argument");
  const T& t = which ? p->ops[index].y2 : p->ops[index].y;
  DVSR_REQUIRE(t.valid(), DVSR_ERR_INVALID, "edvr_op_output: launch %d has no output %d", index, which);
  *in_arena = t.space == SP_ARENA;
  *offset_floats = (long long)t.off;
  *numel = (long long)t.numel;
  return DVSR_OK;
}

extern "C" int dvsr_edvr_tensor_info(const dvsr_edvr_plan* p, const char* name, long long* offset_floats,
                                     long long* numel) {
  DVSR_REQUIRE(p && name && offset_floats && numel, DVSR_ERR_INVALID, "edvr_tensor_info: null argument");
  for (const auto& kv : p->named)
    if (kv.first == name && kv.second.space == SP_ARENA) {
      *offset_floats = (long long)kv.second.off;
      *numel = (long long)kv.second.numel;
      return DVSR_OK;
    }
  set_error("edvr_tensor_info: no tensor named '%s'", name);
  return DVSR_ERR_INVALID;
}


struct dvsr_edvr_stream {
  dvsr_edvr_plan extract, fuse;
  int slots = 0;
  dvsr::SlotLayout sl;
  size_t fea_off[3] = {0, 0, 0};
};

extern "C" int dvsr_edvr_stream_create(const dvsr_edvr_config* cfg, int H, int W, int slots, dvsr_edvr_stream** out) {
  DVSR_REQUIRE(cfg && out, DVSR_ERR_INVALID, "edvr_stream_create: null argument");
  DVSR_REQUIRE(H > 0 && W > 0 && H % 4 == 0 && W % 4 == 0, DVSR_ERR_INVALID,
               "edvr_stream_create: H=%d W=%d (H, W must be positive multiples of 4)", H, W);
  DVSR_REQUIRE(cfg->nf > 0 && cfg->groups > 0 && cfg->nf % cfg->groups == 0 && cfg->nframes > 0 && cfg->front_RBs >= 0 &&
                   cfg->back_RBs >= 0, DVSR_ERR_INVALID, "edvr_stream_create: bad network config");
  DVSR_REQUIRE(cfg->nframes <= DVSR_STREAM_MAX_FRAMES, DVSR_ERR_UNSUPPORTED, "edvr_stream_create: nframes=%d (at most %d)",
               cfg->nframes, DVSR_STREAM_MAX_FRAMES);
  DVSR_REQUIRE(slots >= cfg->nframes, DVSR_ERR_INVALID, "edvr_stream_create: slots=%d < nframes=%d", slots, cfg->nframes);
  DVSR_REQUIRE(cfg->scale == 4 || cfg->scale == 2, DVSR_ERR_UNSUPPORTED, "edvr_stream_create: scale=%d (2 or 4)", cfg->scale);
  DVSR_REQUIRE(cfg->center >= 0 && cfg->center < cfg->nframes, DVSR_ERR_INVALID, "edvr_stream_create: center=%d out of range",
               cfg->center);
  const int cpg = cfg->nf / cfg->groups;
  DVSR_REQUIRE(cpg == 4 || cpg == 8 || cpg == 16, DVSR_ERR_UNSUPPORTED, "edvr_stream_create: nf/groups=%d (supported: 4, 8, 16)", cpg);
  dvsr_edvr_stream* s = new dvsr_edvr_stream();
  const char* v1 = getenv("DVSR_CONV_V1");
  int k = 0;
  for (dvsr_edvr_plan* p : {&s->extract, &s->fuse}) {
    p->cfg = *cfg; p->B = 1; p->H = H; p->W = W;
    p->use_v1 = v1 && v1[0] == '1';
    int rc = build_plan(*p, k++ == 0 ? PART_EXTRACT : PART_FUSE);
    if (rc != DVSR_OK) { delete s; return rc; }
  }
  s->slots = slots;
  s->sl = slot_layout(cfg->nf, H, W);
  static const char* const names[3] = {"L1_fea", "L2_fea", "L3_fea"};
  for (int l = 0; l < 3; ++l)
    for (const auto& kv : s->fuse.named)
      if (kv.first == names[l]) s->fea_off[l] = kv.second.off;
  *out = s;
  return DVSR_OK;
}

extern "C" void dvsr_edvr_stream_destroy(dvsr_edvr_stream* s) { delete s; }

extern "C" int dvsr_edvr_stream_num_params(const dvsr_edvr_stream* s) { return s ? s->fuse.n_params : -1; }

extern "C" int dvsr_edvr_stream_num_launches(const dvsr_edvr_stream* s, int which) {
  if (!s) return -1;
  return which ? (int)s->fuse.ops.size() + 1 : (int)s->extract.ops.size();
}

extern "C" size_t dvsr_edvr_stream_cache_bytes(const dvsr_edvr_stream* s) {
  return s ? (size_t)s->slots * s->sl.floats * sizeof(float) : 0;
}

extern "C" size_t dvsr_edvr_stream_workspace_bytes(const dvsr_edvr_stream* s) {
  return s ? (s->fuse.arena_floats + s->extract.arena_floats) * sizeof(float) : 0;
}

static int stream_check(const dvsr_edvr_stream* s, const void* params, const void* cache, size_t cache_bytes, const void* ws,
                        size_t ws_bytes, const char* what) {
  DVSR_REQUIRE(s && params && cache && ws, DVSR_ERR_INVALID, "%s: null argument", what);
  DVSR_REQUIRE(cache_bytes >= dvsr_edvr_stream_cache_bytes(s), DVSR_ERR_INVALID, "%s: cache %zu < %zu bytes", what, cache_bytes,
               dvsr_edvr_stream_cache_bytes(s));
  DVSR_REQUIRE(ws_bytes >= dvsr_edvr_stream_workspace_bytes(s), DVSR_ERR_INVALID, "%s: workspace %zu < %zu bytes", what, ws_bytes,
               dvsr_edvr_stream_workspace_bytes(s));
// ... 269 lines not shown
```

### dynavsr_amd/csrc/kernels.h

```cpp
#pragma once
#include "../../include/dynavsr_hip.h"
#include "common.h"

namespace dvsr {

struct ConvExtra {
  int wt = 0;
  int w_ctot = 0, w_coff = 0;
  int in_ps = 0;
  int in_dil = 0, Hs = 0, Ws = 0;
  int accum = 0;
  const float* gmask = nullptr;
  int gmask_act = 0;
  int wdiv = 1; long long w_gs = 0; int b_gs = 0;
};
int conv2d_run(const dvsr_conv2d_desc& d, const ConvExtra& ex, hipStream_t st);

int mdcn_forward_run(const float* x, const float* off, long long off_bs, const float* msk,
                     long long msk_bs, int mask_logit, const float* w, const float* b, float* out,
                     int N, int C, int H, int W, int Cout, int kh, int kw, int stride, int pad,
                     int dil, int groups, int dg, int act, hipStream_t st);

enum class ConvKernel : int {
  REG = 0,
  DMA_HALO = 1,
  ROW_SPLIT = 2,
  WINO_F2 = 3,
  WINO_F2_BF16 = 4,
  WINO_F4 = 5,
};
enum class PackLayout : int {
  INTERLEAVED = 0,
  DMA_ORDER = 1,
  ROW_SPLIT = 2,
  WINO_F2 = 3,
  WINO_F2_BF16 = 4,
  WINO_F4 = 5,
  DCN_SPLIT = 6,
};
constexpr PackLayout pack_layout(ConvKernel k) { return static_cast<PackLayout>(static_cast<int>(k)); }
constexpr bool is_winograd(ConvKernel k) { return k == ConvKernel::WINO_F2 || k == ConvKernel::WINO_F2_BF16 || k == ConvKernel::WINO_F4; }
constexpr bool on_bf16_split(ConvKernel k) { return k == ConvKernel::WINO_F2_BF16 || k == ConvKernel::WINO_F4; }
constexpr bool needs_dma_halo_inputs(ConvKernel k) { return k == ConvKernel::DMA_HALO || is_winograd(k); }
constexpr double multiplies_per_output_ratio(ConvKernel k) { return k == ConvKernel::WINO_F4 ? 0.25 : (is_winograd(k) ? 16.0 / 36.0 : 1.0); }
constexpr const char* kernel_tag(ConvKernel k) {
  return k == ConvKernel::WINO_F4 ? "w5" : (k == ConvKernel::WINO_F2_BF16 ? "w3" : (k == ConvKernel::WINO_F2 ? "w" : (k == ConvKernel::REG ? "" : "d")));
}
constexpr bool has_own_pack_kernel(PackLayout l) { return static_cast<int>(l) >= static_cast<int>(PackLayout::WINO_F2); }

struct PackEntry {
  const float* w; float* P;
  int Cout, Ctot, KK, CC, wt, w_ctot, w_coff, ncb, nchunks, pch;
  int bf = 0;
  PackLayout layout = PackLayout::INTERLEAVED;
};
struct PackTable {
  int n;
  PackEntry e[48];
};
int pack_weights_run(const PackTable& t, hipStream_t st);
struct ConvGeo { int cc, th, mt; int bf = 0; ConvKernel kernel = ConvKernel::REG; };
enum ConvAllow : int {
  ALLOW_NONE = 0,
  ALLOW_KSPLIT = 1,
  ALLOW_DMA_HALO = 2,
  ALLOW_WINO = 4,
  ALLOW_WINO_F4 = 8,
  ALLOW_SHARED_DEVICE = 16,
  ALLOW_ONLY_F4 = 32,
};
constexpr ConvAllow operator|(ConvAllow a, ConvAllow b) { return static_cast<ConvAllow>(static_cast<int>(a) | static_cast<int>(b)); }
constexpr ConvAllow without(ConvAllow a, ConvAllow b) { return static_cast<ConvAllow>(static_cast<int>(a) & ~static_cast<int>(b)); }
ConvGeo conv2_choose(int ks, int stride, int N, int Ho, int Wo, int Cout, int Ctot, ConvAllow allow = ALLOW_KSPLIT);
size_t conv2_pack_floats(int ks, int Cout, int Ctot, int cc, int bf, PackLayout layout);
PackEntry conv2_pack_entry(const float* w, float* P, int ks, int Cout, int Ctot, int cc, int bf, PackLayout layout, int wt = 0,
                           int w_ctot = 0, int w_coff = 0);
inline size_t conv2_pack_floats(int ks, int Cout, int Ctot, const ConvGeo& g) {
  return conv2_pack_floats(ks, Cout, Ctot, g.cc, g.bf, pack_layout(g.kernel));
}
inline PackEntry conv2_pack_entry(const float* w, float* P, int ks, int Cout, int Ctot, const ConvGeo& g, int wt = 0, int w_ctot = 0,
                                  int w_coff = 0) {
  return conv2_pack_entry(w, P, ks, Cout, Ctot, g.cc, g.bf, pack_layout(g.kernel), wt, w_ctot, w_coff);
}
double conv2_f4_occupied_cycles(int N, int Ho, int Wo, int Cout, int Ctot, int th);
int pack_weights_wino_run(const PackTable& t, hipStream_t st);
int pack_weights_wino3_run(const PackTable& t, hipStream_t st);
int pack_weights_wino5_run(const PackTable& t, hipStream_t st);
int conv2d_packed_run(const dvsr_conv2d_desc& d, const float* wp, const ConvExtra& ex, const ConvGeo& geo,
                      hipStream_t st);

bool conv1x1_dual_ok(const float* x, const float* w0, const float* w1, const float* y0, const float* y1, int Cin, long long HW);
int conv1x1_dual_run(const float* x, const float* w0, const float* b0, const float* w1, const float* b1, float* y0, float* y1,
                     int N, int Cin, int HW, int act, hipStream_t st, int wdiv = 1, long long w_gs = 0, int b_gs = 0);
int conv3x3_small_cout_run(const float* x, const float* w, const float* bias, const float* res, float* y, int N,
                           int C, int H, int W, int Cout, int act, hipStream_t st, int wdiv = 1, long long w_gs = 0,
                           int b_gs = 0);

struct WgradReduceEntry {
  float* partial; float* dbp; float* dW; float* db;
  int nslot, KK, OP, CP, Cout, Cin, Ctot, c_off;
  int ngroups = 1;
  long long dW_gs = 0, db_gs = 0;
};
constexpr int WGRAD_REDUCE_BATCH = 44;
struct WgradReduceTable {
  int n;
  WgradReduceEntry e[WGRAD_REDUCE_BATCH];
};
int wgrad_reduce_batch(const WgradReduceEntry* entries, int n, hipStream_t st, int blocks = 96);
struct WgradDesc {
  const float* x = nullptr; long long x_bs = 0; int x_bdiv = 1;
  const float* gy = nullptr; int gy_ps = 0;
  float* dW = nullptr; float* db = nullptr;
  int N = 0, Cin = 0, H = 0, W = 0, Cout = 0, Ctot = 0, c_off = 0, ks = 0, stride = 1, pad = -1;
  int groups = 1; long long dW_gs = 0, db_gs = 0;
  int mode = 0;
};
enum class WgradKernel : int {
  SIMPLE = 0,
  PIPE = 1,
  BF16 = 2,
  SPLIT_SCALAR = 3,
  SPLIT_VECTOR = 4,
  SPLIT_WAVE8 = 5,
};
constexpr bool on_bf16_pipe(WgradKernel k) { return k >= WgradKernel::BF16; }
constexpr bool on_bf16_split(WgradKernel k) { return k >= WgradKernel::SPLIT_SCALAR; }
struct WgradGeo {
  WgradKernel kernel = WgradKernel::PIPE;
  int row_split = 0;
  int vx = 0;
  int nsplit = 1, nslot = 1;
  dim3 grid; int block = 256;
};
WgradGeo conv2d_wgrad_choose(const WgradDesc& d);
bool wgrad_split3_default();
size_t conv2d_wgrad_workspace_bytes(const WgradDesc& d);
int conv2d_wgrad_run(const WgradDesc& d, void* ws, size_t ws_bytes, hipStream_t st, int scratch_is_zero = 0,
                     WgradReduceEntry* defer = nullptr);
size_t mdcn_backward_workspace_bytes(int N, int C, int H, int W, int Cout, int stride, int pad, int dil, int groups = 1);
int mdcn_backward_run(const float* x, const float* off, long long off_bs, const float* msk, long long msk_bs,
                      int mask_logit, const float* w, const float* gout, float* gx, float* goff,
                      long long goff_bs, float* gmsk, long long gmsk_bs, float* gw, float* gb, int N, int C,
                      int H, int W, int Cout, int stride, int pad, int dil, int dg, void* ws,
                      size_t ws_bytes, hipStream_t st, int groups = 1, long long gw_gs = 0, long long gb_gs = 0,
                      long long w_gs = 0);

int mdcn_forward_packed_run(const float* x, const float* off, long long off_bs, const float* msk,
                            long long msk_bs, int mask_logit, const float* wp, const float* b, float* out,
                            int N, int C, int H, int W, int Cout, int dg, int act, hipStream_t st, int wdiv = 1,
                            long long w_gs = 0, int b_gs = 0, PackLayout layout = PackLayout::INTERLEAVED);
int mdcn_fwd_variant();
int mdcn_pack_floats();
PackLayout mdcn_pack_layout(int W);
int pack_weights_dcn3_run(const PackTable& t, hipStream_t st);

struct DcnK2 {
  const float* x; const float* off; const float* msk; const float* wp; const float* bias; float* out;
  long long off_bstride, msk_bstride;
  int mask_logit;
  int N, C, H, W, Cout, dg, act;
  int tiles_x, tiles_y, ntiles, ncb, nchunks;
  int wdiv = 1; long long w_gs = 0; int b_gs = 0;
#ifdef DVSR_CONV_TRACE
  long long* trace;
#endif
};
int mdcn_fwd_split_launch(const DcnK2& k, int grid, int mask_logit, hipStream_t st);

int upsample_bilinear_fwd(const float* x, float* y, size_t planes, int H, int W, int S, float mul,
                          hipStream_t st);
int upsample_bilinear_bwd(const float* gy, float* gx, size_t planes, int H, int W, int S, float mul,
                          int accumulate, hipStream_t st);
int pool3s2_fwd(const float* x, float* ymax, float* yavg, size_t planes, int H, int W, hipStream_t st);
int pool3s2_bwd(const float* x, const float* gmax, const float* gavg, float* gx, size_t planes,
                int H, int W, int accumulate, hipStream_t st);
int reduce_frames(float* dst, long long dst_bs, const float* src, int B, int cnt, size_t per,
                  int accumulate, hipStream_t st);
int tsa_gate_fwd(const float* emb, const float* emb_ref, const float* aligned, float* cor,
                 float* gated, int B, int N, int C, size_t HW, hipStream_t st);
int tsa_gate_bwd(const float* emb, const float* emb_ref, const float* aligned, const float* cor,
                 const float* g_gated, float* g_emb, float* g_emb_ref, float* g_aligned, int B,
                 int N, int C, size_t HW, hipStream_t st, float* gdot_scratch = nullptr);
int tsa_blend_fwd(const float* fea, const float* att, const float* add, float* out, size_t n,
                  hipStream_t st);
int tsa_blend_bwd(const float* fea, const float* att, const float* g, float* g_fea, float* g_att_io,
                  size_t n, int accumulate, hipStream_t st);
int add_inplace(float* dst, const float* src, size_t n, hipStream_t st);
int add_out(float* y, const float* a, const float* b, size_t n, hipStream_t st);
int act_bwd_inplace(float* g, const float* y, size_t n, int act, hipStream_t st);

int stream_gather_run(const float* cache, size_t slot_floats, const size_t src_off[3], float* const dst[3],
                      const size_t level_floats[3], int nframes, const int* slots, hipStream_t st);

hipStream_t side_stream_for(hipStream_t st, bool* known = nullptr);

int frame_ingest_check(const char* what, const void* src, const dvsr_frame_desc* sd, const float* dst, int Hp, int Wp,
                       int pad_mode);
int frame_ingest_launch(const void* src, const dvsr_frame_desc& sd, float* dst, int Hp, int Wp, int pad_mode, hipStream_t st);

struct Yuv420 {
  void* plane[3];
  long long rs[3];
  int h, w, matrix, range;
  bool semi;
  int bytes, depth;
};
int yuv420_from(const char* what, const dvsr_yuv_desc* d, Yuv420* f);
int yuv420_from(const char* what, const dvsr_yuv16_desc* d, Yuv420* f);
int frame_ingest_yuv_check(const char* what, const Yuv420& f, const float* dst, int Hp, int Wp, int pad_mode);
int frame_ingest_yuv_launch(const Yuv420& f, float* dst, int Hp, int Wp, int pad_mode, hipStream_t st);

enum : int { PAD_REFLECT = 0, PAD_REFLECT_S2D = 1, PAD_REPL_T3 = 2 };
size_t pad_out_numel(int mode, size_t N, int C, int H, int W);
int pad_fwd(const float* x, float* y, int mode, int N, int C, int H, int W, int T, hipStream_t st);
int pad_bwd(const float* gy, float* gx, int mode, int N, int C, int H, int W, int T, int accumulate,
            hipStream_t st, const float* gmask = nullptr, int gmask_act = 0, int gmask_padded = 0);
int meansub_slices();
int meansub_fwd(const float* x, float* xm, float* mean, float* part, int B, int C, int T, int H, int W,
                hipStream_t st);
int addmean_fwd(const float* y, const float* mean, float* out, int B, int C, int T, size_t HW, hipStream_t st);
int addmean_bwd(const float* gout, float* gy, int B, int C, int T, size_t HW, hipStream_t st);
int w4_to_s2d(const float* w, float* w2, int Cout, int C, int inverse, hipStream_t st);

__device__ __forceinline__ float sigmoidf_(float v) { return 1.f / (1.f + expf(-v)); }

struct DcnTap {
  int o1, o2, o3, o4;
  float w1, w2, w3, w4;
  float lh, lw;
  bool v1, v2, v3, v4;
};

__device__ __forceinline__ bool make_tap(float h_im, float w_im, int H, int W, DcnTap& t) {
  if (!(h_im > -1.f && w_im > -1.f && h_im < (float)H && w_im < (float)W)) return false;
  const int h_lo = (int)floorf(h_im), w_lo = (int)floorf(w_im);
  const int h_hi = h_lo + 1, w_hi = w_lo + 1;
  t.lh = h_im - (float)h_lo;
  t.lw = w_im - (float)w_lo;
  const float hh = 1.f - t.lh, hw = 1.f - t.lw;
  t.v1 = h_lo >= 0 && w_lo >= 0;
  t.v2 = h_lo >= 0 && w_hi <= W - 1;
  t.v3 = h_hi <= H - 1 && w_lo >= 0;
  t.v4 = h_hi <= H - 1 && w_hi <= W - 1;
  t.o1 = t.v1 ? h_lo * W + w_lo : 0;
  t.o2 = t.v2 ? h_lo * W + w_hi : 0;
  t.o3 = t.v3 ? h_hi * W + w_lo : 0;
  t.o4 = t.v4 ? h_hi * W + w_hi : 0;
  t.w1 = hh * hw; t.w2 = hh * t.lw; t.w3 = t.lh * hw; t.w4 = t.lh * t.lw;
  return true;
}

}
```

### dynavsr_amd/csrc/misc.hip

```cpp
#include <cstdint>
#include <cstdlib>

#include "common.h"
#include "kernels.h"

namespace dvsr {

static inline int stream_grid(size_t n, int block = 256) {
  size_t g = (n + block - 1) / block;
  const size_t cap = 256 * 16;
  return (int)(g < cap ? (g ? g : 1) : cap);
}

__device__ __forceinline__ void src_index(int dst, float inv_scale, int in_size, int& i0, int& i1,
                                          float& l1) {
  float s = ((float)dst + 0.5f) * inv_scale - 0.5f;
  s = s < 0.f ? 0.f : s;
  i0 = (int)s;
  i1 = i0 + (i0 < in_size - 1 ? 1 : 0);
  l1 = s - (float)i0;
}

__global__ void upsample_bilinear_fwd_kernel(const float* __restrict__ x, float* __restrict__ y,
                                             size_t planes, int H, int W, int S, float mul) {
  const int Ho = H * S, Wo = W * S;
  const size_t total = planes * Ho * Wo;
  const float inv = 1.f / (float)S;
  for (size_t i = blockIdx.x * (size_t)blockDim.x + threadIdx.x; i < total;
       i += (size_t)gridDim.x * blockDim.x) {
    const int ox = (int)(i % Wo);
    const size_t t = i / Wo;
    const int oy = (int)(t % Ho);
    const size_t p = t / Ho;
    int y0, y1, x0, x1;
    float ly, lx;
    src_index(oy, inv, H, y0, y1, ly);
    src_index(ox, inv, W, x0, x1, lx);
    const float* pl = x + p * (size_t)H * W;
    const float v = (1.f - ly) * ((1.f - lx) * pl[y0 * W + x0] + lx * pl[y0 * W + x1]) +
                    ly * ((1.f - lx) * pl[y1 * W + x0] + lx * pl[y1 * W + x1]);
    y[i] = v * mul;
  }
}

__global__ void upsample_bilinear_fwd4_kernel(const float* __restrict__ x, float* __restrict__ y,
                                              unsigned planes, int H, int W, int S, float mul) {
  const int Ho = H * S, Wo = W * S, Wq = Wo >> 2;
  const unsigned total = planes * (unsigned)Ho * (unsigned)Wq;
  const float inv = 1.f / (float)S;
  for (unsigned i = blockIdx.x * blockDim.x + threadIdx.x; i < total; i += gridDim.x * blockDim.x) {
    const int oq = (int)(i % (unsigned)Wq);
    const unsigned t = i / (unsigned)Wq;
    const int oy = (int)(t % (unsigned)Ho);
    const unsigned p = t / (unsigned)Ho;
    int y0, y1;
    float ly;
    src_index(oy, inv, H, y0, y1, ly);
    const float* r0 = x + (size_t)p * H * W + (size_t)y0 * W;
    const float* r1 = x + (size_t)p * H * W + (size_t)y1 * W;
    f32x4 out;
#pragma unroll
    for (int j = 0; j < 4; ++j) {
      int x0, x1;
      float lx;
      src_index(4 * oq + j, inv, W, x0, x1, lx);
      out[j] = ((1.f - ly) * ((1.f - lx) * r0[x0] + lx * r0[x1]) + ly * ((1.f - lx) * r1[x0] + lx * r1[x1])) * mul;
    }
    *reinterpret_cast<f32x4*>(y + ((size_t)p * Ho + oy) * Wo + 4 * oq) = out;
  }
}

__global__ void upsample2x_fwd_kernel(const float* __restrict__ x, float* __restrict__ y, unsigned planes, int H,
                                      int W, float mul) {
  const int Wq = W >> 2, Wo = 2 * W;
  const unsigned total = planes * (unsigned)H * (unsigned)Wq;
  for (unsigned i = blockIdx.x * blockDim.x + threadIdx.x; i < total; i += gridDim.x * blockDim.x) {
    const int xq = (int)(i % (unsigned)Wq);
    const unsigned t = i / (unsigned)Wq;
    const int iy = (int)(t % (unsigned)H);
    const unsigned p = t / (unsigned)H;
    const float* pl = x + (size_t)p * H * W;
    const int x0 = 4 * xq;
    const int rows[3] = {iy > 0 ? iy - 1 : 0, iy, iy < H - 1 ? iy + 1 : H - 1};
    float h[3][8];
#pragma unroll
    for (int r = 0; r < 3; ++r) {
      const float* row = pl + (size_t)rows[r] * W;
      const f32x4 c = *reinterpret_cast<const f32x4*>(row + x0);
      const float in[6] = {row[x0 > 0 ? x0 - 1 : 0], c[0], c[1], c[2], c[3], row[x0 + 4 < W ? x0 + 4 : W - 1]};
#pragma unroll
      for (int j = 0; j < 4; ++j) {
        h[r][2 * j] = (x0 + j > 0) ? 0.25f * in[j] + 0.75f * in[j + 1] : in[j + 1];
        h[r][2 * j + 1] = 0.75f * in[j + 1] + 0.25f * in[j + 2];
      }
    }
    float* o0 = y + ((size_t)p * 2 * H + 2 * iy) * Wo + 2 * x0;
    f32x4 a0, a1, b0, b1;
#pragma unroll
    for (int j = 0; j < 8; ++j) {
      const float ev = iy > 0 ? 0.25f * h[0][j] + 0.75f * h[1][j] : h[1][j];
      const float od = 0.75f * h[1][j] + 0.25f * h[2][j];
      if (j < 4) { a0[j] = ev * mul; b0[j] = od * mul; } else { a1[j - 4] = ev * mul; b1[j - 4] = od * mul; }
    }
    *reinterpret_cast<f32x4*>(o0) = a0;
    *reinterpret_cast<f32x4*>(o0 + 4) = a1;
    *reinterpret_cast<f32x4*>(o0 + Wo) = b0;
    *reinterpret_cast<f32x4*>(o0 + Wo + 4) = b1;
  }
}

__global__ void upsample2x_fwd2_kernel(const float* __restrict__ x, float* __restrict__ y, unsigned planes, int H,
                                       int W, float mul) {
  const int Wh = W >> 1, Wo = 2 * W;
  const unsigned total = planes * (unsigned)H * (unsigned)Wh;
  for (unsigned i = blockIdx.x * blockDim.x + threadIdx.x; i < total; i += gridDim.x * blockDim.x) {
    const int xh = (int)(i % (unsigned)Wh);
    const unsigned t = i / (unsigned)Wh;
    const int iy = (int)(t % (unsigned)H);
    const unsigned p = t / (unsigned)H;
    const float* pl = x + (size_t)p * H * W;
    const int x0 = 2 * xh;
    const int rows[3] = {iy > 0 ? iy - 1 : 0, iy, iy < H - 1 ? iy + 1 : H - 1};
    float h[3][4];
#pragma unroll
    for (int r = 0; r < 3; ++r) {
      const float* row = pl + (size_t)rows[r] * W;
      typedef float f32x2_ __attribute__((ext_vector_type(2)));
      const f32x2_ c = *reinterpret_cast<const f32x2_*>(row + x0);
      const float in[4] = {row[x0 > 0 ? x0 - 1 : 0], c[0], c[1], row[x0 + 2 < W ? x0 + 2 : W - 1]};
#pragma unroll
      for (int j = 0; j < 2; ++j) {
        h[r][2 * j] = (x0 + j > 0) ? 0.25f * in[j] + 0.75f * in[j + 1] : in[j + 1];
        h[r][2 * j + 1] = 0.75f * in[j + 1] + 0.25f * in[j + 2];
      }
    }
    float* o0 = y + ((size_t)p * 2 * H + 2 * iy) * Wo + 2 * x0;
    f32x4 a0, b0;
#pragma unroll
    for (int j = 0; j < 4; ++j) {
      const float ev = iy > 0 ? 0.25f * h[0][j] + 0.75f * h[1][j] : h[1][j];
      const float od = 0.75f * h[1][j] + 0.25f * h[2][j];
      a0[j] = ev * mul; b0[j] = od * mul;
    }
    *reinterpret_cast<f32x4*>(o0) = a0;
    *reinterpret_cast<f32x4*>(o0 + Wo) = b0;
  }
}

__global__ void upsample_bilinear_bwd_kernel(const float* __restrict__ gy, float* __restrict__ gx,
                                             size_t planes, int H, int W, int S, float mul,
                                             int accumulate) {
  const int Ho = H * S, Wo = W * S;
  const size_t total = planes * H * W;
  const float inv = 1.f / (float)S;
  for (size_t i = blockIdx.x * (size_t)blockDim.x + threadIdx.x; i < total;
       i += (size_t)gridDim.x * blockDim.x) {
    const int ix = (int)(i % W);
    const size_t t = i / W;
    const int iy = (int)(t % H);
    const size_t p = t / H;
    const float* g = gy + p * (size_t)Ho * Wo;
    float acc = 0.f;
    const int oy_lo = max(0, (iy - 1) * S), oy_hi = min(Ho, (iy + 2) * S);
    const int ox_lo = max(0, (ix - 1) * S), ox_hi = min(Wo, (ix + 2) * S);
    for (int oy = oy_lo; oy < oy_hi; ++oy) {
      int y0, y1;
      float ly;
      src_index(oy, inv, H, y0, y1, ly);
      float wy = 0.f;
      if (y0 == iy) wy += 1.f - ly;
      if (y1 == iy) wy += ly;
      if (wy == 0.f) continue;
      for (int ox = ox_lo; ox < ox_hi; ++ox) {
        int x0, x1;
        float lx;
        src_index(ox, inv, W, x0, x1, lx);
        float wx = 0.f;
        if (x0 == ix) wx += 1.f - lx;
        if (x1 == ix) wx += lx;
        if (wx != 0.f) acc += wy * wx * g[(size_t)oy * Wo + ox];
      }
    }
    acc *= mul;
    gx[i] = accumulate ? gx[i] + acc : acc;
  }
}

__global__ void pool3s2_fwd_kernel(const float* __restrict__ x, float* __restrict__ ymax,
                                   float* __restrict__ yavg, size_t planes, int H, int W, int Ho,
                                   int Wo) {
  const size_t total = planes * Ho * Wo;
  for (size_t i = blockIdx.x * (size_t)blockDim.x + threadIdx.x; i < total;
       i += (size_t)gridDim.x * blockDim.x) {
    const int ox = (int)(i % Wo);
    const size_t t = i / Wo;
    const int oy = (int)(t % Ho);
    const size_t p = t / Ho;
    const float* pl = x + p * (size_t)H * W;
    float mx = -INFINITY, sum = 0.f;
#pragma unroll
    for (int dy = -1; dy <= 1; ++dy) {
      const int yy = 2 * oy + dy;
      if ((unsigned)yy >= (unsigned)H) continue;
#pragma unroll
      for (int dx = -1; dx <= 1; ++dx) {
        const int xx = 2 * ox + dx;
        if ((unsigned)xx >= (unsigned)W) continue;
        const float v = pl[yy * W + xx];
        mx = fmaxf(mx, v);
        sum += v;
      }
    }
    ymax[i] = mx;
    yavg[i] = sum * (1.f / 9.f);
  }
}

__global__ void pool3s2_bwd_kernel(const float* __restrict__ x, const float* __restrict__ gmax,
                                   const float* __restrict__ gavg, float* __restrict__ gx,
                                   size_t planes, int H, int W, int Ho, int Wo, int accumulate) {
// ... 603 lines not shown
```

### dynavsr_amd/engine.py

```python
import ctypes
import threading

import torch

from . import _lib as L

_plans = {}
_GEOMETRY_ENV = ("DVSR_CONV_WINO", "DVSR_CONV_WINO3", "DVSR_CONV_WINO5", "DVSR_CONV_V1", "DVSR_EST_SPLIT", "DVSR_EST_SPLIT2", "DVSR_FUSE_ACT_BWD",
                 "DVSR_BWD_STREAMS", "DVSR_PCD_HOIST")
_PROCESS_ENV = ("DVSR_CONV_LDS", "DVSR_CONV_LAST_MFMA", "DVSR_SPLIT_TH8_FROM", "DVSR_WGRAD_SPLIT3",
                "DVSR_WGRAD_WIDE", "DVSR_WGRAD_S3V", "DVSR_WGRAD_S3_KYS_BELOW", "DVSR_WGRAD_S3_WGS", "DVSR_WGRAD_S3W", "DVSR_DCN_FWD", "DVSR_DCN_BWD",
                "DVSR_EST_FUSE_PAD", "DVSR_FUSE_RES_BWD", "DVSR_BWD_FORK_EVERY", "DVSR_BWD_PROBE", "DVSR_TSA_DUAL", "DVSR_TSA_V",
                "DVSR_DEGRADE_GENERIC", "DVSR_UP2")
_process_env_seen = None


def _check_process_env():
    import os
    import warnings
    global _process_env_seen
    now = tuple(os.environ.get(k) for k in _PROCESS_ENV)
    if _process_env_seen is None:
        _process_env_seen = now
        return
    for k, a, b in zip(_PROCESS_ENV, _process_env_seen, now):
        if a != b:
            warnings.warn("dynavsr_amd: %s=%r now, but the native library read %r when the first plan of this process was built "
                          "and keeps that value (switches of this kind are read once per process: set them before the first "
                          "plan, one process per value)" % (k, b, a), RuntimeWarning, stacklevel=3)
    _process_env_seen = now


_WORK_KEYS = ("fwd_algorithmic", "fwd_executed", "bwd_algorithmic", "bwd_executed", "fwd_bytes",
              "fwd_f32_pipe", "fwd_bf16_pipe", "bwd_f32_pipe", "bwd_bf16_pipe")


def _env_key():
    import os
    return tuple(os.environ.get(k) for k in _GEOMETRY_ENV)


class Plan:

    def __init__(self, cfg, b, h, w, grad_groups=1, weight_sets=1):
        self.key = (cfg, b, h, w, grad_groups, weight_sets)
        cfg = tuple(cfg) + (0,) * (8 - len(cfg))
        self.cfg = dict(zip(("nf", "nframes", "groups", "front_RBs", "back_RBs", "scale", "center", "bf16_mfma"), cfg))
        self.b, self.h, self.w, self.grad_groups, self.weight_sets = b, h, w, grad_groups, weight_sets
        self._h = ctypes.c_void_p()
        L.check(L.lib().dvsr_edvr_plan_create_ex(L.EdvrConfig(*cfg), b, h, w, grad_groups, weight_sets,
                                                 ctypes.byref(self._h)), "dvsr_edvr_plan_create_ex")
        self.n_params = L.lib().dvsr_edvr_num_params(self._h)
        self.n_launches = L.lib().dvsr_edvr_num_launches(self._h)
        self.n_backward_launches = L.lib().dvsr_edvr_num_backward_launches(self._h)

    def workspace_bytes(self, need_grad):
        return int(L.lib().dvsr_edvr_workspace_bytes(self._h, int(need_grad)))

    def forward(self, params, x, out, ws, packed=False):
        arr = (ctypes.c_void_p * len(params))(*[L.ptr(p) for p in params])
        fn = L.lib().dvsr_edvr_forward_packed if packed else L.lib().dvsr_edvr_forward
        L.check(fn(self._h, arr, L.ptr(x), L.ptr(out), ws.data_ptr(), ws.numel() * ws.element_size(), L.stream()),
                "dvsr_edvr_forward_packed" if packed else "dvsr_edvr_forward")

    def backward(self, params, x, gout, gparams, gx, ws):
        arr = (ctypes.c_void_p * len(params))(*[L.ptr(p) for p in params])
        garr = (ctypes.c_void_p * len(gparams))(*[L.ptr(g) for g in gparams])
        L.check(L.lib().dvsr_edvr_backward(self._h, arr, L.ptr(x), L.ptr(gout), garr, L.ptr(gx),
                                           ws.data_ptr(), ws.numel() * ws.element_size(), L.stream()),
                "dvsr_edvr_backward")

    def forward_timed(self, params, x, out, ws):
        arr = (ctypes.c_void_p * len(params))(*[L.ptr(p) for p in params])
        ms = (ctypes.c_float * self.n_launches)()
        L.check(L.lib().dvsr_edvr_forward_timed(self._h, arr, L.ptr(x), L.ptr(out), ws.data_ptr(),
                                                ws.numel() * ws.element_size(), L.stream(), ms),
                "dvsr_edvr_forward_timed")
        return list(ms)

    def work(self, nograd=False):
        out = (ctypes.c_double * 9)()
        fn = L.lib().dvsr_edvr_plan_work_nograd if nograd else L.lib().dvsr_edvr_plan_work
        L.check(fn(self._h, ctypes.byref(out)), "dvsr_edvr_plan_work")
        return dict(zip(_WORK_KEYS, out))

    def op_output(self, ws, index, which=0):
        ia, off, n = ctypes.c_int(), ctypes.c_longlong(), ctypes.c_longlong()
        L.check(L.lib().dvsr_edvr_op_output(self._h, index, which, ctypes.byref(ia), ctypes.byref(off), ctypes.byref(n)),
                "dvsr_edvr_op_output")
        if not ia.value:
            return None
        return ws.view(torch.float32)[off.value:off.value + n.value]

    def op_info(self):
        out = []
        kind, name = ctypes.create_string_buffer(32), ctypes.create_string_buffer(64)
        fl, by = ctypes.c_double(), ctypes.c_double()
        for i in range(self.n_launches):
            L.check(L.lib().dvsr_edvr_op_info(self._h, i, kind, 32, name, 64, ctypes.byref(fl),
                                              ctypes.byref(by)), "dvsr_edvr_op_info")
            out.append((kind.value.decode(), name.value.decode(), fl.value, by.value))
        return out

    def tensor(self, ws, name, shape=None):
        off, n = ctypes.c_longlong(), ctypes.c_longlong()
        L.check(L.lib().dvsr_edvr_tensor_info(self._h, name.encode(), ctypes.byref(off),
                                              ctypes.byref(n)), "dvsr_edvr_tensor_info")
        t = ws.view(torch.float32)[off.value:off.value + n.value]
        return t.view(shape) if shape is not None else t

    def __del__(self):
        try:
            if self._h:
                L.lib().dvsr_edvr_plan_destroy(self._h)
        except Exception:
            pass


def get_plan(cfg, b, h, w, device=None, grad_groups=1, weight_sets=1):
    dev = torch.cuda.current_device() if device is None else torch.device(device).index
    key = (tuple(cfg), b, h, w, dev, torch.cuda.current_stream(dev).cuda_stream, grad_groups, weight_sets, _env_key())
    p = _plans.get(key)
    if p is None:
        _check_process_env()
        p = _plans[key] = Plan(tuple(cfg), b, h, w, grad_groups, weight_sets)
    return p


def _stash(ctx, plan, ws, x, params):
    ctx.plan, ctx.ws, ctx.x, ctx.params = plan, ws, x, params
    ctx.versions = [p._version for p in params]


def _check_stash(ctx, what):
    if ctx.ws is None:
        raise RuntimeError("%s: backward called a second time -- the activation arena was released after the "
                           "first one (the tape is first-order and single-use, like once_differentiable in "
                           "deform_conv.py:123)" % what)
    for i, (p, v) in enumerate(zip(ctx.params, ctx.versions)):
        if p._version != v:
            raise RuntimeError("%s: parameter %d was modified in place between forward and backward (version %d -> "
                               "%d); the gradient would be taken at the wrong weights" % (what, i, v, p._version))


def _prep(t):
    if t.dtype != torch.float32:
        t = t.float()
    return t.contiguous()


_grad_mode = threading.local()


class _TapeFunction(torch.autograd.Function):

    @classmethod
    def apply(cls, *args, **kwargs):
        _grad_mode.enabled = torch.is_grad_enabled()
        return super().apply(*args, **kwargs)


def _need_grad(ctx):
    return bool(getattr(_grad_mode, "enabled", True)) and any(ctx.needs_input_grad)
# ... 369 lines not shown
```

### include/dynavsr_hip.h

```cpp
#ifndef DYNAVSR_HIP_H_
#define DYNAVSR_HIP_H_

#include <stddef.h>

#ifdef __cplusplus
extern "C" {
#endif

#define DVSR_OK 0
#define DVSR_ERR_INVALID (-1)
#define DVSR_ERR_UNSUPPORTED (-2)
#define DVSR_ERR_WORKSPACE (-3)
#define DVSR_ERR_HIP (-4)

#define DVSR_ACT_NONE 0
#define DVSR_ACT_LRELU 1
#define DVSR_ACT_RELU 2

typedef void* dvsr_stream_t;

const char* dvsr_last_error(void);
int dvsr_version(void);

int dvsr_mdcn_forward(const float* x, const float* offset, const float* mask, const float* w,
// ... 141 lines not shown
#define DVSR_FRAME_U16_Y_10 5
#define DVSR_FRAME_U16_Y_12 6
int dvsr_frame_luma_sad(const void* a, const void* b, const dvsr_frame_desc* desc, long long frame_stride, int pairs,
                        unsigned long long* sad, dvsr_stream_t stream);

#define DVSR_YUV_NV12 0
#define DVSR_YUV_I420 1
#define DVSR_YUV_BT601 0
#define DVSR_YUV_BT709 1
#define DVSR_YUV_LIMITED 0
#define DVSR_YUV_FULL 1
typedef struct dvsr_yuv_desc {
  int format;
  int h, w;
  int matrix, range;
  void* plane[3];
  long long row_stride[3];
} dvsr_yuv_desc;
int dvsr_frame_ingest_yuv(const dvsr_yuv_desc* sd, float* dst, int Hp, int Wp, int pad_mode, dvsr_stream_t stream);
int dvsr_frame_emit_yuv(const float* src, int Hs, int Ws, const dvsr_yuv_desc* dd, float lo, float hi, dvsr_stream_t stream);
int dvsr_edvr_stream_extract_frame_yuv(const dvsr_edvr_stream* stream_plan, const float* const* params, const dvsr_yuv_desc* fd,
                                       int pad_mode, int slot, void* cache, size_t cache_bytes, void* workspace,
                                       size_t workspace_bytes, int packed, dvsr_stream_t stream);

#define DVSR_YUV16_SEMI_MSB 0
#define DVSR_YUV16_PLANAR_LSB 1
typedef struct dvsr_yuv16_desc {
  int format, depth;
  int h, w;
  int matrix, range;
  void* plane[3];
  long long row_stride[3];
} dvsr_yuv16_desc;
int dvsr_frame_ingest_yuv16(const dvsr_yuv16_desc* sd, float* dst, int Hp, int Wp, int pad_mode, dvsr_stream_t stream);
int dvsr_frame_emit_yuv16(const float* src, int Hs, int Ws, const dvsr_yuv16_desc* dd, float lo, float hi, dvsr_stream_t stream);
int dvsr_edvr_stream_extract_frame_yuv16(const dvsr_edvr_stream* stream_plan, const float* const* params,
                                         const dvsr_yuv16_desc* fd, int pad_mode, int slot, void* cache, size_t cache_bytes,
                                         void* workspace, size_t workspace_bytes, int packed, dvsr_stream_t stream);

typedef struct dvsr_resize_axis {
  const int* first;
  const float* weights;
  int taps;
} dvsr_resize_axis;
int dvsr_frame_resize_taps(int n_in, int n_out);
int dvsr_frame_resize_table(int n_in, int n_out, int taps, int* first, float* weights);
int dvsr_frame_resize(const float* src, int Hs, int Ws, int h, int w, float* dst, int Ho, int Wo, int oh, int ow,
                      const dvsr_resize_axis* rows, const dvsr_resize_axis* cols, dvsr_stream_t stream);

#define DVSR_FLIP_W 1
#define DVSR_FLIP_H 2
int dvsr_frame_flip(const float* src, float* dst, long long planes, int H, int W, int flags, dvsr_stream_t stream);
int dvsr_frame_flip_mean(const float* y0, const float* yw, const float* yh, const float* yhw, float* dst,
                         long long planes, int H, int W, dvsr_stream_t stream);

#define DVSR_ESTIMATOR_MFDN 0
#define DVSR_ESTIMATOR_SFDN 1
typedef struct dvsr_estimator_config {
  int kind;
  int nf;
  int in_nc;
  int scale;
  int nframes;
} dvsr_estimator_config;
typedef struct dvsr_estimator_plan dvsr_estimator_plan;
int dvsr_estimator_plan_create(const dvsr_estimator_config* cfg, int B, int H, int W, dvsr_estimator_plan** out);
int dvsr_estimator_plan_create_grouped(const dvsr_estimator_config* cfg, int B, int H, int W, int grad_groups,
                                       dvsr_estimator_plan** out);
int dvsr_estimator_plan_create_ex(const dvsr_estimator_config* cfg, int B, int H, int W, int grad_groups, int weight_sets,
                                  dvsr_estimator_plan** out);
void dvsr_estimator_plan_destroy(dvsr_estimator_plan* plan);
int dvsr_estimator_num_params(const dvsr_estimator_plan* plan);
int dvsr_estimator_num_launches(const dvsr_estimator_plan* plan, int backward);
int dvsr_estimator_plan_work(const dvsr_estimator_plan* plan, double* out9);
size_t dvsr_estimator_workspace_bytes(const dvsr_estimator_plan* plan, int need_grad);
int dvsr_estimator_forward(const dvsr_estimator_plan* plan, const float* const* params, const float* x, float* out,
                           void* workspace, size_t workspace_bytes, dvsr_stream_t stream);
int dvsr_estimator_backward(const dvsr_estimator_plan* plan, const float* const* params, const float* x,
                            const float* grad_out, float* const* grad_params, void* workspace,
                            size_t workspace_bytes, dvsr_stream_t stream);

size_t dvsr_charbonnier_workspace_bytes(void);
int dvsr_charbonnier_forward(const float* x, const float* y, float* loss, long long n, float eps,
                             void* workspace, size_t workspace_bytes, dvsr_stream_t stream);
int dvsr_charbonnier_backward(const float* x, const float* y, const float* grad_loss, float* gx, long long n,
                              float eps, dvsr_stream_t stream);
int dvsr_charbonnier_forward_grouped(const float* x, const float* y, float* loss, long long n, int groups, float eps,
                                     void* workspace, size_t workspace_bytes, dvsr_stream_t stream);
int dvsr_charbonnier_backward_grouped(const float* x, const float* y, const float* grad_loss, float* gx, long long n,
                                      int groups, float eps, dvsr_stream_t stream);

int dvsr_l1_tail_forward(const float* x, const float* y, const float* base, float weight, float* loss, long long n,
                         void* workspace, size_t workspace_bytes, dvsr_stream_t stream);
int dvsr_l1_tail_backward(const float* x, const float* y, const float* grad_loss, float weight, float* gx, long long n,
                          dvsr_stream_t stream);
int dvsr_l1_tail_forward_grouped(const float* x, const float* y, const float* base, float weight, float* loss, long long n,
                                 int groups, void* workspace, size_t workspace_bytes, dvsr_stream_t stream);
int dvsr_l1_tail_backward_grouped(const float* x, const float* y, const float* grad_loss, float weight, float* gx,
                                  long long n, int groups, dvsr_stream_t stream);

size_t dvsr_conv2d_packed_workspace_bytes(const dvsr_conv2d_desc* d);
int dvsr_conv2d_forward_packed(const dvsr_conv2d_desc* d, void* workspace, size_t workspace_bytes, dvsr_stream_t stream);
int dvsr_conv2d_dgrad_packed(const dvsr_conv2d_desc* d, const float* gy, float* gx0, void* workspace,
                             size_t workspace_bytes, dvsr_stream_t stream);
int dvsr_conv2d_packed_geometry(const dvsr_conv2d_desc* d, int geo[4]);

int dvsr_conv2d_wgrad_bf16(const dvsr_conv2d_desc* d, const float* gy, float* gw, float* gb, void* workspace,
                           size_t workspace_bytes, dvsr_stream_t stream);
int dvsr_conv2d_wgrad_split3(const dvsr_conv2d_desc* d, const float* gy, float* gw, float* gb, void* workspace,
                             size_t workspace_bytes, dvsr_stream_t stream);

int dvsr_conv2d_wgrad_geometry(const dvsr_conv2d_desc* d, int mode, int groups, int geo[8]);
size_t dvsr_conv2d_wgrad_workspace_bytes(const dvsr_conv2d_desc* d, int groups);

int dvsr_flow_warp_forward(const float* x, const float* flow, float* out, int N, int C, int H, int W,
                           long long out_bstride, dvsr_stream_t stream);
int dvsr_flow_warp_backward(const float* x, const float* flow, const float* grad_out, float* grad_x, float* grad_flow,
                            int N, int C, int H, int W, long long gout_bstride, dvsr_stream_t stream);
int dvsr_avgpool2_forward(const float* x, float* y, long long planes, int H, int W, dvsr_stream_t stream);
int dvsr_avgpool2_backward(const float* grad_y, float* grad_x, long long planes, int H, int W, int accumulate,
                           dvsr_stream_t stream);
int dvsr_resize_bilinear_ac_forward(const float* x, float* y, long long planes, int H, int W, int Ho, int Wo, float mul,
                                    long long y_plane_stride, dvsr_stream_t stream);
int dvsr_resize_bilinear_ac_backward(const float* grad_y, float* grad_x, long long planes, int H, int W, int Ho, int Wo,
                                     float mul, long long gy_plane_stride, dvsr_stream_t stream);
int dvsr_upsample_bicubic_ac_forward(const float* x, float* y, long long planes, int H, int W, int scale,
                                     dvsr_stream_t stream);
int dvsr_upsample_bicubic_ac_backward(const float* grad_y, float* grad_x, long long planes, int H, int W, int scale,
                                      dvsr_stream_t stream);
int dvsr_channel_affine(const float* x, const float* scale, const float* shift, float* out, int N, int C, long long HW,
                        long long x_bstride, long long out_bstride, int accumulate, dvsr_stream_t stream);
size_t dvsr_batchnorm_workspace_bytes(int C);
int dvsr_batchnorm_forward(const float* x, const float* gamma, const float* beta, float* running_mean,
                           float* running_var, float* y, float* save_mean, float* save_rstd, int N, int C, long long HW,
                           int training, float momentum, float eps, int relu, void* workspace, size_t workspace_bytes,
                           dvsr_stream_t stream);
int dvsr_batchnorm_backward(const float* x, const float* grad_y, const float* y, const float* gamma,
                            const float* save_mean, const float* save_rstd, float* grad_x, float* grad_gamma,
                            float* grad_beta, int N, int C, long long HW, int training, int relu, void* workspace,
                            size_t workspace_bytes, dvsr_stream_t stream);

int dvsr_temporal_gather3_forward(const float* x, float* y, int B, int T, int C, long long HW, int pad_t,
                                  dvsr_stream_t stream);
int dvsr_temporal_gather3_backward(const float* grad_y, float* grad_x, int B, int T, int C, long long HW, int pad_t,
                                   dvsr_stream_t stream);
int dvsr_dynamic_filter_forward(const float* x_center, const float* filter_logits, const float* residual, float* out,
                                int B, int H, int W, int scale, int adapt_official, dvsr_stream_t stream);
int dvsr_dynamic_filter_backward(const float* x_center, const float* filter_logits, const float* grad_out,
                                 float* grad_logits, float* grad_residual, float* grad_x_center, int B, int H, int W,
                                 int scale, int adapt_official, dvsr_stream_t stream);

int dvsr_conv3x3_small_cout(const float* x, const float* w, const float* bias, const float* res, float* y, int N, int C, int H,
                            int W, int Cout, int act, dvsr_stream_t stream);

int dvsr_conv1x1_dual(const float* x, const float* w0, const float* b0, const float* w1, const float* b1, float* y0, float* y1,
                      int N, int Cin, int H, int W, int act, dvsr_stream_t stream);

int dvsr_patch_gather_forward(const float* src, float* dst, const int* py, const int* px, int P, int planes, int H, int W,
                              int edge, int scale, dvsr_stream_t stream);
int dvsr_patch_gather_backward(const float* grad_dst, float* grad_src, const int* py, const int* px, int P, int planes,
                               int H, int W, int edge, int scale, dvsr_stream_t stream);

int dvsr_adam_step(float* const* params, const float* const* grads, float* const* exp_avg,
                   float* const* exp_avg_sq, const long long* numel, int n_tensors, float lr, float beta1,
                   float beta2, float eps, float weight_decay, int step, dvsr_stream_t stream);
int dvsr_sgd_step(float* const* params, const float* const* grads, const long long* numel, int n_tensors,
                  float lr, float weight_decay, dvsr_stream_t stream);
int dvsr_replicate_tensors(const float* const* src, float* const* dst, const long long* numel, int n_tensors, int copies,
                           dvsr_stream_t stream);

size_t dvsr_frame_metrics_workspace_bytes(int C, int H, int W);
int dvsr_frame_metrics(const float* sr, const float* gt, int C, int H, int W, float lo, float hi,
                       unsigned char* sr_hwc_u8, double* out, void* workspace, size_t workspace_bytes,
                       dvsr_stream_t stream);

int dvsr_degrade_apply(const float* img, const float* kernels, float* out, int N, int C, int H, int W, int K,
                       int scale, int n_kernels, int kernel_offset, int quantise, dvsr_stream_t stream);

#ifdef __cplusplus
}
#endif
#endif
```

Measured before the change: 269.4 frames/s.

## Fuse bilinear base upsample into conv_last MFMA epilogue with persistent banded tiles

In no-grad forward mode, the final 64->3 conv now computes the bilinear-upsampled base frame directly in its epilogue, reading the low-res input. The separate base upsample op is skipped, which removes the write and re-read of a full HR base tensor. The MFMA small-Cout kernel becomes persistent: it walks tiles in bands and prefetches the next tile's halo while computing the current one. The MFMA path is now on by default (previously opt-in), and the bilinear helper is shared with contraction turned off to match the standalone kernel numerically.

```diff
diff --git a/dynavsr_amd/_lib.py b/dynavsr_amd/_lib.py
--- a/dynavsr_amd/_lib.py
+++ b/dynavsr_amd/_lib.py
@@ -163,6 +163,7 @@
         "dvsr_dynamic_filter_forward": (I, [P, P, P, P, I, I, I, I, I, P]),
         "dvsr_dynamic_filter_backward": (I, [P, P, P, P, P, P, I, I, I, I, I, P]),
         "dvsr_conv3x3_small_cout": (I, [P, P, P, P, P, I, I, I, I, I, I, P]),
+        "dvsr_conv3x3_small_cout_base": (I, [P, P, P, P, P, I, I, I, I, I, I, I, P]),
         "dvsr_conv1x1_dual": (I, [P, P, P, P, P, P, P, I, I, I, I, I, P]),
         "dvsr_patch_gather_forward": (I, [P, P, POINTER(c_int), POINTER(c_int), I, I, I, I, I, I, P]),
         "dvsr_patch_gather_backward": (I, [P, P, POINTER(c_int), POINTER(c_int), I, I, I, I, I, I, P]),
diff --git a/dynavsr_amd/csrc/conv_small.hip b/dynavsr_amd/csrc/conv_small.hip
--- a/dynavsr_amd/csrc/conv_small.hip
+++ b/dynavsr_amd/csrc/conv_small.hip
@@ -1,3 +1,6 @@
+#include <algorithm>
+#include <cstdlib>
+
 #include "common.h"
 #include "kernels.h"
 
@@ -7,6 +10,7 @@
   const float* x; const float* w; const float* bias; const float* res; float* y;
   int N, C, H, W, Cout, act, tiles_x, tiles_y, ntiles;
   int wdiv; long long w_gs; int b_gs;
+  int bands; const float* lr; int lrS; long long lr_bs;
 };
 
 typedef float f32x2 __attribute__((ext_vector_type(2)));
@@ -134,102 +138,135 @@
   return __builtin_bit_cast(f32x4, __builtin_amdgcn_raw_buffer_load_b128(rs, (int)voff, (int)soff, 0));
 }
 
-template <int COUT>
+template <int COUT, bool BASE>
 __global__ __launch_bounds__(256, 2) void conv3x3_small_cout_mfma_kernel(SmallK a) {
   using Sh = SmallMfmaShape;
   constexpr int TH = Sh::TH, TW = Sh::TW, RW = Sh::RW, NPOS = Sh::NPOS, AP = Sh::APITCH, NM = 9 * COUT;
   extern __shared__ __attribute__((aligned(16))) float s_mf[];
   float* const s_a = s_mf;
   float* const s_p = s_mf + 32 * AP;
-  const int tpx = (a.ntiles + 7) >> 3;
-  const int tile = (blockIdx.x & 7) * tpx + (blockIdx.x >> 3);
-  if ((int)(blockIdx.x >> 3) >= tpx || tile >= a.ntiles) return;
-  const int tx_ = tile % a.tiles_x;
-  const int t2 = tile / a.tiles_x;
-  const int ty_ = t2 % a.tiles_y;
-  const int n = t2 / a.tiles_y;
-  const int oy0 = ty_ * TH, ox0 = tx_ * TW;
+  const int wpb = gridDim.x / a.bands, band = blockIdx.x % a.bands, tpb = (a.ntiles + a.bands - 1) / a.bands;
+  const int tend = min((band + 1) * tpb, a.ntiles);
+  int tile = band * tpb + (int)(blockIdx.x / a.bands);
+  if (tile >= tend) return;
   const int tid = threadIdx.x, lane = tid & 63;
   const int wave = __builtin_amdgcn_readfirstlane(tid >> 6);
   const int nn = lane & 31, kk = lane >> 5;
   const unsigned HW4 = (unsigned)a.H * a.W * 4u;
+  const size_t HW = (size_t)a.H * a.W;
+
+  const int hrow = 2 * wave + (nn >> 4) - 1, hcol = 4 * (nn & 15) - Sh::X0;
+  auto halo_voff = [&](int oy0, int ox0) __attribute__((always_inline)) {
+    const int gy = oy0 + hrow, gx = ox0 + hcol;
+    const bool inimg = (unsigned)gy < (unsigned)a.H && (unsigned)gx < (unsigned)a.W;
+    return inimg ? (unsigned)(8 * kk) * HW4 + (unsigned)(gy * a.W + gx) * 4u : 0x80000000u;
+  };
+  f32x4 B[2][16];
+  auto issue = [&](int half, __amdgpu_buffer_rsrc_t rs, unsigned voff) __attribute__((always_inline)) {
+#pragma unroll
+    for (int s = 0; s < 16; ++s) {
+      const int c = 16 * (2 * half + (s >> 3)) + (s & 7);
+      B[half][s] = sm_load16(rs, voff, (unsigned)c * HW4);
+    }
+  };
+  int tx_ = tile % a.tiles_x, t2 = tile / a.tiles_x;
+  int n = t2 / a.tiles_y, oy0 = (t2 - n * a.tiles_y) * TH, ox0 = tx_ * TW;
   const float* wn = wset_ptr(a.w, a.w_gs, n, a.wdiv);
   const float* bn = wset_ptr(a.bias, a.b_gs, n, a.wdiv);
-
-  const int gy = oy0 - 1 + 2 * wave + (nn >> 4), gx = ox0 - Sh::X0 + 4 * (nn & 15);
-  const bool inimg = (unsigned)gy < (unsigned)a.H && (unsigned)gx < (unsigned)a.W;
-  const unsigned voff = inimg ? (unsigned)(8 * kk) * HW4 + (unsigned)(gy * a.W + gx) * 4u : 0x80000000u;
-  const __amdgpu_buffer_rsrc_t xrs = sm_rsrc(a.x + (size_t)n * 64 * a.H * a.W);
-  f32x4 B[2][16];
-  auto issue = [&](int half) __attribute__((always_inline)) {
-#pragma unroll
-    for (int s = 0; s < 16; ++s) {
-      const int c = 16 * (2 * half + (s >> 3)) + (s & 7);
-      B[half][s] = sm_load16(xrs, voff, (unsigned)c * HW4);
-    }
-  };
-  issue(0);
-  for (int i = tid; i < 32 * 64; i += 256) {
-    const int m = i >> 6, c = i & 63;
-    const int tap = m / COUT, o = m - tap * COUT;
-    s_a[m * AP + c] = m < NM ? wn[((size_t)o * 64 + c) * 9 + tap] : 0.f;
-  }
-  issue(1);
+  {
+    const __amdgpu_buffer_rsrc_t rs = sm_rsrc(a.x + (size_t)n * 64 * HW);
+    const unsigned voff = halo_voff(oy0, ox0);
+    issue(0, rs, voff);
+    for (int i = tid; i < 32 * 64; i += 256) {
+      const int m = i >> 6, c = i & 63;
+      const int tap = m / COUT, o = m - tap * COUT;
+      s_a[m * AP + c] = m < NM ? wn[((size_t)o * 64 + c) * 9 + tap] : 0.f;
+    }
+    issue(1, rs, voff);
+  }
   __syncthreads();
   f32x4 A[8];
 #pragma unroll
   for (int q = 0; q < 8; ++q) A[q] = *reinterpret_cast<const f32x4*>(s_a + nn * AP + 16 * (q >> 1) + 8 * kk + 4 * (q & 1));
-
-  f32x16 acc[4];
-#pragma unroll
-  for (int j = 0; j < 4; ++j)
-#pragma unroll
-    for (int r = 0; r < 16; ++r) acc[j][r] = 0.f;
-#pragma unroll
-  for (int half = 0; half < 2; ++half)
-#pragma unroll
-    for (int s = 0; s < 16; ++s) {
-      const int ch = 2 * half + (s >> 3), i = s & 7;
-      const float av = A[2 * ch + (i >> 2)][i & 3];
-#pragma unroll
-      for (int j = 0; j < 4; ++j) acc[j] = __builtin_amdgcn_mfma_f32_32x32x2f32(av, B[half][s][j], acc[j], 0, 0, 0);
-    }
-
-#pragma unroll
-  for (int r = 0; r < 16; ++r) {
-    const int m = (r & 3) + 8 * (r >> 2) + 4 * kk;
-    if (m < NM)
-      *reinterpret_cast<f32x4*>(s_p + m * NPOS + 128 * wave + 4 * nn) = f32x4{acc[0][r], acc[1][r], acc[2][r], acc[3][r]};
-  }
-  __syncthreads();
-
-  if (tid >= TH * (TW / 2)) return;
-  const int y = tid / (TW / 2), xp = (tid - y * (TW / 2)) * 2;
-  const int oy = oy0 + y, ox = ox0 + xp;
-  if (oy >= a.H || ox >= a.W) return;
-  float s0[COUT], s1[COUT];
-#pragma unroll
-  for (int o = 0; o < COUT; ++o) { s0[o] = 0.f; s1[o] = 0.f; }
-#pragma unroll
-  for (int dy = 0; dy < 3; ++dy) {
-    const float* row = s_p + (y + dy) * RW + xp + Sh::X0 - 1;
-#pragma unroll
-    for (int dx = 0; dx < 3; ++dx)
+  float bvs[COUT];
+#pragma unroll
+  for (int o = 0; o < COUT; ++o) bvs[o] = bn ? bn[o] : 0.f;
+  const int sy = tid / (TW / 2), sxp = (tid - sy * (TW / 2)) * 2;
+  const float inv = BASE ? 1.f / (float)a.lrS : 0.f;
+  const int lrH = BASE ? a.H / a.lrS : 0, lrW = BASE ? a.W / a.lrS : 0;
+
+  for (;;) {
+    const int tnext = tile + wpb;
+    const bool more = tnext < tend;
+    const int ntx = tnext % a.tiles_x, nt2 = tnext / a.tiles_x;
+    const int nn_ = nt2 / a.tiles_y, noy0 = (nt2 - nn_ * a.tiles_y) * TH, nox0 = ntx * TW;
+    const __amdgpu_buffer_rsrc_t nrs = sm_rsrc(a.x + (size_t)(more ? nn_ : n) * 64 * HW);
+    const unsigned nvoff = more ? halo_voff(noy0, nox0) : 0x80000000u;
+
+    f32x16 acc[4];
+#pragma unroll
+    for (int j = 0; j < 4; ++j)
+#pragma unroll
+      for (int r = 0; r < 16; ++r) acc[j][r] = 0.f;
+#pragma unroll
+    for (int half = 0; half < 2; ++half) {
+#pragma unroll
+      for (int s = 0; s < 16; ++s) {
+        const int ch = 2 * half + (s >> 3), i = s & 7;
+        const float av = A[2 * ch + (i >> 2)][i & 3];
+#pragma unroll
+        for (int j = 0; j < 4; ++j) acc[j] = __builtin_amdgcn_mfma_f32_32x32x2f32(av, B[half][s][j], acc[j], 0, 0, 0);
+      }
+      issue(half, nrs, nvoff);
+    }
+
+    __syncthreads();
+#pragma unroll
+    for (int r = 0; r < 16; ++r) {
+      const int m = (r & 3) + 8 * (r >> 2) + 4 * kk;
+      if (m < NM)
+        *reinterpret_cast<f32x4*>(s_p + m * NPOS + 128 * wave + 4 * nn) = f32x4{acc[0][r], acc[1][r], acc[2][r], acc[3][r]};
+    }
+    __syncthreads();
+
+    const int oy = oy0 + sy, ox = ox0 + sxp;
+    if (tid < TH * (TW / 2) && oy < a.H && ox < a.W) {
+      float s0[COUT], s1[COUT];
+#pragma unroll
+      for (int o = 0; o < COUT; ++o) { s0[o] = 0.f; s1[o] = 0.f; }
+#pragma unroll
+      for (int dy = 0; dy < 3; ++dy) {
+        const float* row = s_p + (sy + dy) * RW + sxp + Sh::X0 - 1;
+#pragma unroll
+        for (int dx = 0; dx < 3; ++dx)
+#pragma unroll
+          for (int o = 0; o < COUT; ++o) {
+            const float* pm = row + ((dy * 3 + dx) * COUT + o) * NPOS + dx;
+            s0[o] += pm[0];
+            s1[o] += pm[1];
+          }
+      }
+      int by0 = 0, by1 = 0;
+      float bly = 0.f;
+      if (BASE) src_index(oy, inv, lrH, by0, by1, bly);
 #pragma unroll
       for (int o = 0; o < COUT; ++o) {
-        const float* pm = row + ((dy * 3 + dx) * COUT + o) * NPOS + dx;
-        s0[o] += pm[0];
-        s1[o] += pm[1];
-      }
-  }
-  const size_t HW = (size_t)a.H * a.W;
-#pragma unroll
-  for (int o = 0; o < COUT; ++o) {
-    const float bv = bn ? bn[o] : 0.f;
-    f32x2 v = {apply_act(s0[o] + bv, a.act), apply_act(s1[o] + bv, a.act)};
-    const size_t idx = ((size_t)n * a.Cout + o) * HW + (size_t)oy * a.W + ox;
-    if (a.res) v += *reinterpret_cast<const f32x2*>(a.res + idx);
-    *reinterpret_cast<f32x2*>(a.y + idx) = v;
+        const float bv = bvs[o];
+        f32x2 v = {apply_act(s0[o] + bv, a.act), apply_act(s1[o] + bv, a.act)};
+        const size_t idx = ((size_t)n * a.Cout + o) * HW + (size_t)oy * a.W + ox;
+        if (BASE) {
+          const float* pl = a.lr + (size_t)n * a.lr_bs + (size_t)o * lrH * lrW;
+          const float* r0 = pl + (size_t)by0 * lrW;
+          const float* r1 = pl + (size_t)by1 * lrW;
+          v += f32x2{bilinear_out(r0, r1, bly, ox, inv, lrW, 1.f), bilinear_out(r0, r1, bly, ox + 1, inv, lrW, 1.f)};
+        } else if (a.res) {
+          v += *reinterpret_cast<const f32x2*>(a.res + idx);
+        }
+        *reinterpret_cast<f32x2*>(a.y + idx) = v;
+      }
+    }
+    if (!more) break;
+    tile = tnext; n = nn_; oy0 = noy0; ox0 = nox0;
   }
 }
 
@@ -237,22 +274,43 @@
 static int launch_small_mfma(SmallK k, hipStream_t st) {
   using Sh = SmallMfmaShape;
   k.tiles_x = ceil_div(k.W, Sh::TW); k.tiles_y = ceil_div(k.H, Sh::TH); k.ntiles = k.tiles_x * k.tiles_y * k.N;
-  auto kern = conv3x3_small_cout_mfma_kernel<COUT>;
-  static PerDeviceOnce once;
-  set_dyn_lds_once(once, (const void*)kern, Sh::LDS_BYTES);
-  hipLaunchKernelGGL(kern, dim3(8 * ceil_div(k.ntiles, 8)), dim3(256), Sh::LDS_BYTES, st, k);
+  int cap = 2 * device_cus();
+  if (const char* v = getenv("DVSR_CONV_LAST_WGS")) { const int c = atoi(v); if (c > 0) cap = c; }
+  const int g = std::min(k.ntiles, cap);
+  k.bands = std::min(8, g);
+  const int tpb = ceil_div(k.ntiles, k.bands);
+  const int wpb = k.w_gs ? tpb : std::min(tpb, g / k.bands);
+  auto kern = k.lr ? conv3x3_small_cout_mfma_kernel<COUT, true> : conv3x3_small_cout_mfma_kernel<COUT, false>;
+  static PerDeviceOnce once[2];
+  set_dyn_lds_once(once[k.lr ? 1 : 0], (const void*)kern, Sh::LDS_BYTES);
+  hipLaunchKernelGGL(kern, dim3(k.bands * wpb), dim3(256), Sh::LDS_BYTES, st, k);
   return check_launch("conv3x3_small_cout_mfma_kernel");
 }
 
+static bool small_mfma_on() {
+  const char* v = getenv("DVSR_CONV_LAST_MFMA");
+  return !(v && v[0] == '0');
+}
+static bool small_mfma_ok(const float* x, const float* y, const float* res, int C, int H, int W, int Cout, long long w_gs) {
+  return C == 64 && Cout >= 1 && Cout <= 3 && W % 4 == 0 && (unsigned long long)C * H * W * 4 < 0x7fffffffull &&
+         ((((uintptr_t)x | (uintptr_t)y | (uintptr_t)res) & 15) == 0) && w_gs % 4 == 0;
+}
+bool conv3x3_small_cout_fuses_base(const float* x, const float* y, const float* lr, int C, int H, int W, int Cout, long long w_gs,
+                                   int lr_scale) {
+  return lr && lr_scale >= 1 && H % lr_scale == 0 && W % lr_scale == 0 && small_mfma_on() && small_mfma_ok(x, y, nullptr, C, H, W, Cout, w_gs);
+}
+
 int conv3x3_small_cout_run(const float* x, const float* w, const float* bias, const float* res, float* y, int N,
-                           int C, int H, int W, int Cout, int act, hipStream_t st, int wdiv, long long w_gs, int b_gs) {
+                           int C, int H, int W, int Cout, int act, hipStream_t st, int wdiv, long long w_gs, int b_gs,
+                           const float* lr, int lr_scale, long long lr_bs) {
   DVSR_REQUIRE(x && w && y && Cout >= 1 && Cout <= 4, DVSR_ERR_INVALID, "conv3x3_small_cout: bad argument");
+  DVSR_REQUIRE(!lr || (!res && conv3x3_small_cout_fuses_base(x, y, lr, C, H, W, Cout, w_gs, lr_scale)), DVSR_ERR_UNSUPPORTED,
+               "conv3x3_small_cout: the base frame is computed in the epilogue of the matrix-pipe form only (C=%d Cout=%d W=%d)", C, Cout, W);
   SmallK k;
   k.x = x; k.w = w; k.bias = bias; k.res = res; k.y = y; k.N = N; k.C = C; k.H = H; k.W = W; k.Cout = Cout; k.act = act;
   k.wdiv = wdiv > 0 ? wdiv : 1; k.w_gs = w_gs; k.b_gs = b_gs;
-  static const bool mfma_on = [] { const char* v = getenv("DVSR_CONV_LAST_MFMA"); return v && v[0] == '1'; }();
-  if (mfma_on && C == 64 && Cout <= 3 && W % 4 == 0 && (unsigned long long)C * H * W * 4 < 0x7fffffffull &&
-      ((((uintptr_t)x | (uintptr_t)y | (uintptr_t)res) & 15) == 0) && w_gs % 4 == 0) {
+  k.bands = 8; k.lr = lr; k.lrS = lr_scale; k.lr_bs = lr_bs;
+  if (small_mfma_on() && small_mfma_ok(x, y, res, C, H, W, Cout, w_gs)) {
     if (Cout == 1) return launch_small_mfma<1>(k, st);
     if (Cout == 2) return launch_small_mfma<2>(k, st);
     return launch_small_mfma<3>(k, st);
@@ -275,3 +333,10 @@
   DVSR_REQUIRE(N > 0 && C > 0 && H > 0 && W > 0, DVSR_ERR_INVALID, "conv3x3_small_cout: empty tensor");
   return dvsr::conv3x3_small_cout_run(x, w, bias, res, y, N, C, H, W, Cout, act, (hipStream_t)stream, 1, 0, 0);
 }
+
+extern "C" int dvsr_conv3x3_small_cout_base(const float* x, const float* w, const float* bias, const float* lr, float* y, int N,
+                                            int C, int H, int W, int Cout, int act, int scale, dvsr_stream_t stream) {
+  DVSR_REQUIRE(N > 0 && C > 0 && H > 0 && W > 0 && lr && scale >= 1, DVSR_ERR_INVALID, "conv3x3_small_cout_base: bad argument");
+  return dvsr::conv3x3_small_cout_run(x, w, bias, nullptr, y, N, C, H, W, Cout, act, (hipStream_t)stream, 1, 0, 0, lr, scale,
+                                      (long long)Cout * (H / scale) * (W / scale));
+}
diff --git a/dynavsr_amd/csrc/engine.hip b/dynavsr_amd/csrc/engine.hip
--- a/dynavsr_amd/csrc/engine.hip
+++ b/dynavsr_amd/csrc/engine.hip
@@ -34,6 +34,9 @@
   struct T ypad;
   int fused_into = -1;
   int dual = -1;
+  int base_first = -1, base_conv = -1, lr_scale = 0;
+  struct T lr;
+  long long lr_bs = 0;
   long long x0_bs = 0, x1_bs = 0;
   int S = 1;
   float mul = 1.f;
@@ -411,6 +414,7 @@
   h *= 2; w *= 2;
   out = b.conv("HRconv", b.take(), out, 64, none, 0, B, h, w, 64, 3, 1, L);
   T base = b.alloc("base", (size_t)B * 3 * h * w);
+  const int base_first = (int)p.ops.size();
   for (int bi = 0; bi < B; ++bi) {
     Op o; o.type = OP_UP; o.name = "base_up";
     o.x0 = Builder::view(xin, part == PART_FUSE ? 0 : ((size_t)bi * Nf + ctr) * 3 * HW, 3 * HW);
@@ -420,6 +424,16 @@
   }
   T yout; yout.space = SP_OUTPUT; yout.off = 0; yout.numel = (size_t)B * 3 * h * w;
   b.conv("conv_last", b.take(), out, 64, none, 0, B, h, w, 3, 3, 1, NO, base, 0, 1, 0, 0, yout);
+  {
+    const char* v = getenv("DVSR_CONV_LAST_BASE");
+    if (!(v && v[0] == '0') && !p.use_v1) {
+      const int ic = (int)p.ops.size() - 1;
+      Op& cl = p.ops[ic];
+      cl.base_first = base_first; cl.lr_scale = c.scale;
+      cl.lr = p.ops[base_first].x0; cl.lr_bs = part == PART_FUSE ? 0 : (long long)Nf * 3 * HW;
+      for (int bi = 0; bi < B; ++bi) p.ops[base_first + bi].base_conv = ic;
+    }
+  }
   p.n_params = b.pcur;
   return DVSR_OK;
 }
@@ -854,6 +868,12 @@
   return d;
 }
 
+static bool base_in_epilogue(const dvsr_edvr_plan& p, const Op& cl, const Bases& bs) {
+  return bs.mode == FWD_NOGRAD && cl.type == OP_CONV && cl.base_first >= 0 &&
+         conv3x3_small_cout_fuses_base(bs.at(cl.x0), bs.at(cl.y), bs.at(cl.lr), cl.c0, cl.H, cl.W, cl.Cout,
+                                       p.wsets > 1 ? (long long)cl.Cout * cl.c0 * 9 : 0, cl.lr_scale);
+}
+
 static int run_forward_op(const dvsr_edvr_plan& p, const Op& o, const float* const* P, const Bases& bs, hipStream_t st) {
   switch (o.type) {
     case OP_CONV: {
@@ -882,10 +902,12 @@
       if (o.wmap) d.w = bs.arena + o.w2_off;
       d.x1_bdiv = o.x1_bdiv; d.x0_bstride = o.x0_bs; d.x1_bstride = o.x1_bs;
       if (p.use_v1) return conv2d_run(d, ConvExtra(), st);
-      if (o.Cout <= 4 && o.ks == 3 && o.stride == 1 && !o.c1 && !o.ps && !o.x0_bs && o.pad < 0)
-        return conv3x3_small_cout_run(d.x0, d.w, d.bias, d.res, d.y, o.N, o.c0, o.H, o.W, o.Cout, o.act, st,
+      if (o.Cout <= 4 && o.ks == 3 && o.stride == 1 && !o.c1 && !o.ps && !o.x0_bs && o.pad < 0) {
+        const bool own_base = base_in_epilogue(p, o, bs);
+        return conv3x3_small_cout_run(d.x0, d.w, d.bias, own_base ? nullptr : d.res, d.y, o.N, o.c0, o.H, o.W, o.Cout, o.act, st,
                                       p.wsets > 1 ? o.N / p.wsets : 1, p.wsets > 1 ? (long long)o.Cout * o.c0 * 9 : 0,
-                                      p.wsets > 1 ? o.Cout : 0);
+                                      p.wsets > 1 ? o.Cout : 0, own_base ? bs.at(o.lr) : nullptr, o.lr_scale, o.lr_bs);
+      }
       for (const Op::Launch& l : o.launches[bs.mode]) {
         ConvExtra ex;
         set_wsets(p, o.N, l.pack.floats, o.Cout, &ex);
@@ -907,6 +929,7 @@
                               1, 1, o.dg, o.act, st);
     }
     case OP_UP:
+      if (o.base_conv >= 0 && base_in_epilogue(p, p.ops[o.base_conv], bs)) return DVSR_OK;
       return upsample_bilinear_fwd(bs.at(o.x0), bs.at(o.y), o.planes, o.H, o.W, o.S, o.mul, st);
     case OP_POOL:
       return pool3s2_fwd(bs.at(o.x0), bs.at(o.y), bs.at(o.y2), o.planes, o.H, o.W, st);
@@ -1141,15 +1164,17 @@
   return run_forward_tape(*p, params, Bases{(float*)ws, x, out, forward_mode(p, ws_bytes)}, packs_valid, (hipStream_t)stream);
 }
 
-static void op_work(const Op& o, const char** kind, double* flops, double* bytes) {
+static void op_work(const Op& o, const char** kind, double* flops, double* bytes, FwdMode mode) {
   *flops = 0; *bytes = 0; *kind = "other";
   switch (o.type) {
     case OP_CONV: {
       const int Ho = conv_out(o, o.H), Wo = conv_out(o, o.W);
       const double ctot = o.c0 + o.c1, px = (double)o.N * Ho * Wo;
+      const bool own_base = mode == FWD_NOGRAD && o.base_first >= 0;
       *flops = 2.0 * px * o.Cout * ctot * o.ks * o.ks;
       *bytes = 4.0 * ((double)o.N * o.c0 * o.H * o.W + (double)(o.N / o.x1_bdiv) * o.c1 * o.H * o.W +
-                      px * o.Cout * (o.res.valid() ? 2 : 1) + (double)o.Cout * ctot * o.ks * o.ks);
+                      px * o.Cout * (o.res.valid() && !own_base ? 2 : 1) + (own_base ? px * o.Cout / (o.lr_scale * o.lr_scale) : 0.0) +
+                      (double)o.Cout * ctot * o.ks * o.ks);
       *kind = o.ks == 1 ? "conv1x1" : (o.ks == 2 ? "conv2x2" : (o.stride == 2 ? "conv3x3s2" : "conv3x3s1"));
       break;
     }
@@ -1160,7 +1185,7 @@
       *kind = "mdcn";
       break;
     }
-    case OP_UP: *bytes = 4.0 * o.planes * o.H * o.W * (1.0 + o.S * o.S); *kind = "upsample"; break;
+    case OP_UP: *bytes = (mode == FWD_NOGRAD && o.base_conv >= 0) ? 0.0 : 4.0 * o.planes * o.H * o.W * (1.0 + o.S * o.S); *kind = "upsample"; break;
     case OP_POOL: *bytes = 4.0 * o.planes * o.H * o.W * 1.5; *kind = "pool"; break;
     case OP_GATE: *bytes = 4.0 * ((double)o.gB * o.gN * o.gC * o.gHW * 3 + (double)o.gB * o.gC * o.gHW +
                                  (double)o.gB * o.gN * o.gHW); *kind = "tsa_gate"; break;
@@ -1177,7 +1202,7 @@
   DVSR_REQUIRE(p && kind && name && flops && bytes && index >= 0 && index < (int)p->ops.size(),
                DVSR_ERR_INVALID, "edvr_op_info: bad argument");
   const char* k;
-  op_work(p->ops[index], &k, flops, bytes);
+  op_work(p->ops[index], &k, flops, bytes, FWD_NOGRAD);
   snprintf(kind, kind_cap, "%s", k);
   if (p->ops[index].type == OP_CONV)
   {
@@ -1211,7 +1236,7 @@
   for (const Op& o : p->ops) {
     {
       const char* k; double fl, by;
-      op_work(o, &k, &fl, &by);
+      op_work(o, &k, &fl, &by, mode);
       fby += by;
     }
     if (o.type == OP_CONV) {
diff --git a/dynavsr_amd/csrc/kernels.h b/dynavsr_amd/csrc/kernels.h
--- a/dynavsr_amd/csrc/kernels.h
+++ b/dynavsr_amd/csrc/kernels.h
@@ -94,7 +94,9 @@
                      int N, int Cin, int HW, int act, hipStream_t st, int wdiv = 1, long long w_gs = 0, int b_gs = 0);
 int conv3x3_small_cout_run(const float* x, const float* w, const float* bias, const float* res, float* y, int N,
                            int C, int H, int W, int Cout, int act, hipStream_t st, int wdiv = 1, long long w_gs = 0,
-                           int b_gs = 0);
+                           int b_gs = 0, const float* lr = nullptr, int lr_scale = 0, long long lr_bs = 0);
+bool conv3x3_small_cout_fuses_base(const float* x, const float* y, const float* lr, int C, int H, int W, int Cout, long long w_gs,
+                                   int lr_scale);
 
 struct WgradReduceEntry {
   float* partial; float* dbp; float* dW; float* db;
@@ -225,6 +227,23 @@
 
 __device__ __forceinline__ float sigmoidf_(float v) { return 1.f / (1.f + expf(-v)); }
 
+__device__ __forceinline__ void src_index(int dst, float inv_scale, int in_size, int& i0, int& i1, float& l1) {
+#pragma clang fp contract(off)
+  float s = __builtin_fmaf((float)dst + 0.5f, inv_scale, -0.5f);
+  s = s < 0.f ? 0.f : s;
+  i0 = (int)s;
+  i1 = i0 + (i0 < in_size - 1 ? 1 : 0);
+  l1 = s - (float)i0;
+}
+__device__ __forceinline__ float bilinear_out(const float* r0, const float* r1, float ly, int ox, float inv_scale, int W, float mul) {
+#pragma clang fp contract(off)
+  int x0, x1;
+  float lx;
+  src_index(ox, inv_scale, W, x0, x1, lx);
+  const float t0 = __builtin_fmaf(1.f - lx, r0[x0], lx * r0[x1]), t1 = __builtin_fmaf(1.f - lx, r1[x0], lx * r1[x1]);
+  return __builtin_fmaf(1.f - ly, t0, ly * t1) * mul;
+}
+
 struct DcnTap {
   int o1, o2, o3, o4;
   float w1, w2, w3, w4;
diff --git a/dynavsr_amd/csrc/misc.hip b/dynavsr_amd/csrc/misc.hip
--- a/dynavsr_amd/csrc/misc.hip
+++ b/dynavsr_amd/csrc/misc.hip
@@ -12,14 +12,6 @@
   return (int)(g < cap ? (g ? g : 1) : cap);
 }
 
-__device__ __forceinline__ void src_index(int dst, float inv_scale, int in_size, int& i0, int& i1,
-                                          float& l1) {
-  float s = ((float)dst + 0.5f) * inv_scale - 0.5f;
-  s = s < 0.f ? 0.f : s;
-  i0 = (int)s;
-  i1 = i0 + (i0 < in_size - 1 ? 1 : 0);
-  l1 = s - (float)i0;
-}
 
 __global__ void upsample_bilinear_fwd_kernel(const float* __restrict__ x, float* __restrict__ y,
                                              size_t planes, int H, int W, int S, float mul) {
@@ -60,12 +52,7 @@
     const float* r1 = x + (size_t)p * H * W + (size_t)y1 * W;
     f32x4 out;
 #pragma unroll
-    for (int j = 0; j < 4; ++j) {
-      int x0, x1;
-      float lx;
-      src_index(4 * oq + j, inv, W, x0, x1, lx);
-      out[j] = ((1.f - ly) * ((1.f - lx) * r0[x0] + lx * r0[x1]) + ly * ((1.f - lx) * r1[x0] + lx * r1[x1])) * mul;
-    }
+    for (int j = 0; j < 4; ++j) out[j] = bilinear_out(r0, r1, ly, 4 * oq + j, inv, W, mul);
     *reinterpret_cast<f32x4*>(y + ((size_t)p * Ho + oy) * Wo + 4 * oq) = out;
   }
 }
diff --git a/dynavsr_amd/engine.py b/dynavsr_amd/engine.py
--- a/dynavsr_amd/engine.py
+++ b/dynavsr_amd/engine.py
@@ -7,8 +7,9 @@
 
 _plans = {}
 _GEOMETRY_ENV = ("DVSR_CONV_WINO", "DVSR_CONV_WINO3", "DVSR_CONV_WINO5", "DVSR_CONV_V1", "DVSR_EST_SPLIT", "DVSR_EST_SPLIT2", "DVSR_FUSE_ACT_BWD",
-                 "DVSR_BWD_STREAMS", "DVSR_PCD_HOIST")
-_PROCESS_ENV = ("DVSR_CONV_LDS", "DVSR_CONV_LAST_MFMA", "DVSR_SPLIT_TH8_FROM", "DVSR_WGRAD_SPLIT3",
+                 "DVSR_BWD_STREAMS", "DVSR_PCD_HOIST", "DVSR_CONV_LAST_BASE",
+                 "DVSR_CONV_LAST_MFMA", "DVSR_CONV_LAST_WGS")
+_PROCESS_ENV = ("DVSR_CONV_LDS", "DVSR_SPLIT_TH8_FROM", "DVSR_WGRAD_SPLIT3",
                 "DVSR_WGRAD_WIDE", "DVSR_WGRAD_S3V", "DVSR_WGRAD_S3_KYS_BELOW", "DVSR_WGRAD_S3_WGS", "DVSR_WGRAD_S3W", "DVSR_DCN_FWD", "DVSR_DCN_BWD",
                 "DVSR_EST_FUSE_PAD", "DVSR_FUSE_RES_BWD", "DVSR_BWD_FORK_EVERY", "DVSR_BWD_PROBE", "DVSR_TSA_DUAL", "DVSR_TSA_V",
                 "DVSR_DEGRADE_GENERIC", "DVSR_UP2")
diff --git a/include/dynavsr_hip.h b/include/dynavsr_hip.h
--- a/include/dynavsr_hip.h
+++ b/include/dynavsr_hip.h
@@ -317,6 +317,8 @@
 
 int dvsr_conv3x3_small_cout(const float* x, const float* w, const float* bias, const float* res, float* y, int N, int C, int H,
                             int W, int Cout, int act, dvsr_stream_t stream);
+int dvsr_conv3x3_small_cout_base(const float* x, const float* w, const float* bias, const float* lr, float* y, int N, int C, int H,
+                                 int W, int Cout, int act, int scale, dvsr_stream_t stream);
 
 int dvsr_conv1x1_dual(const float* x, const float* w0, const float* b0, const float* w1, const float* b1, float* y0, float* y1,
                       int N, int Cin, int H, int W, int act, dvsr_stream_t stream);
```

Result: no change. 268.7 frames/s, median of 2 (-0.2%).
